# hongfz16/AvatarCLIP

Measured on NVIDIA H100. Metric: appearance-optim steps/sec (512 rays x 128 samples, CLIP loss), higher is better.
Workload: dtype bf16x3(split)->f32

## Files before the change

### avatarclip_b200/csrc/avc_gemm_tc.cuh

```cuda
#pragma once
#include <type_traits>
#include <cuda.h>
#include <cuda_bf16.h>

#include <cstdlib>

#include "avc_common.cuh"
#include "avc_wgmma.cuh"

namespace avc {
namespace tc {

__device__ __forceinline__ uint32_t smem_u32(const void* p) { return (uint32_t)__cvta_generic_to_shared(p); }

__device__ __forceinline__ void mbar_init(uint32_t bar, uint32_t count) {
  asm volatile("mbarrier.init.shared::cta.b64 [%0], %1;" ::"r"(bar), "r"(count));
}
__device__ __forceinline__ void mbar_expect_tx(uint32_t bar, uint32_t bytes) {
  asm volatile("mbarrier.arrive.expect_tx.shared::cta.b64 _, [%0], %1;" ::"r"(bar), "r"(bytes) : "memory");
}
__device__ __forceinline__ void mbar_arrive(uint32_t bar) {
  asm volatile("mbarrier.arrive.shared::cta.b64 _, [%0];" ::"r"(bar) : "memory");
}
__device__ __forceinline__ void mbar_wait(uint32_t bar, uint32_t parity) {
  uint32_t done = 0;
  for (uint32_t spins = 0; !done; ++spins) {
    asm volatile(
        "{\n\t.reg .pred p;\n\t"
        "mbarrier.try_wait.parity.shared::cta.b64 p, [%1], %2;\n\t"
        "selp.u32 %0, 1, 0, p;\n\t}"
        : "=r"(done) : "r"(bar), "r"(parity) : "memory");
    if (spins > (1u << 26)) __trap();
  }
}
constexpr int kNtProbeSlots = 9;
#ifdef AVC_NT_PROBE
static __device__ unsigned long long g_nt_probe[16][kNtProbeSlots];
#define AVC_PROBE(...) __VA_ARGS__
#define AVC_PROBE_WAIT(acc, bar, par) do { long long t__ = clock64(); mbar_wait(bar, par); (acc) += clock64() - t__; } while (0)
#define AVC_PROBE_ADD(id, slot, v) atomicAdd(&g_nt_probe[id][slot], (unsigned long long)(v))
#else
#define AVC_PROBE(...)
#define AVC_PROBE_WAIT(acc, bar, par) mbar_wait(bar, par)
#define AVC_PROBE_ADD(id, slot, v)
#endif
template <typename E, typename = void>
struct EpiProbeId { static constexpr int value = 0; };
template <typename E>
struct EpiProbeId<E, std::void_t<decltype(E::kProbeId)>> { static constexpr int value = E::kProbeId; };

__device__ __forceinline__ void pdl_wait() { asm volatile("griddepcontrol.wait;" ::: "memory"); }
__device__ __forceinline__ void pdl_trigger() { asm volatile("griddepcontrol.launch_dependents;" ::: "memory"); }
template <typename... KArgs, typename... Args>
static inline cudaError_t launch_pdl(void (*kern)(KArgs...), dim3 grid, dim3 block, size_t smem, cudaStream_t st, Args... args) {
  cudaLaunchConfig_t cfg{};
  cfg.gridDim = grid; cfg.blockDim = block; cfg.dynamicSmemBytes = smem; cfg.stream = st;
  cudaLaunchAttribute at[1];
  at[0].id = cudaLaunchAttributeProgrammaticStreamSerialization;
  at[0].val.programmaticStreamSerializationAllowed = 1;
  const char* e = getenv("AVC_TC_PDL");
  const int on = (e && atoi(e) == 0) ? 0 : 1;
  cfg.attrs = at; cfg.numAttrs = on ? 1 : 0;
  return cudaLaunchKernelEx(&cfg, kern, static_cast<KArgs>(args)...);
}

__device__ __forceinline__ void fence_barrier_init() { asm volatile("fence.mbarrier_init.release.cluster;" ::: "memory"); }
__device__ __forceinline__ void fence_proxy_async() { asm volatile("fence.proxy.async.shared::cta;" ::: "memory"); }
__device__ __forceinline__ void named_bar_sync(int id, int count) {
  asm volatile("bar.sync %0, %1;" ::"r"(id), "r"(count) : "memory");
}
__device__ __forceinline__ void named_bar_arrive(int id, int count) {
  asm volatile("bar.arrive %0, %1;" ::"r"(id), "r"(count) : "memory");
}

__device__ __forceinline__ void tma_load_2d(uint32_t dst, const CUtensorMap* map, int x, int y, uint32_t bar) {
  asm volatile(
      "cp.async.bulk.tensor.2d.shared::cluster.global.tile.mbarrier::complete_tx::bytes [%0], [%1, {%3, %4}], [%2];"
      ::"r"(dst), "l"((uint64_t)map), "r"(bar), "r"(x), "r"(y) : "memory");
}
__device__ __forceinline__ void tma_prefetch_desc(const CUtensorMap* map) {
  asm volatile("prefetch.tensormap [%0];" ::"l"((uint64_t)map) : "memory");
}

typedef CUresult (*PFN_encodeTiled)(CUtensorMap*, CUtensorMapDataType, cuuint32_t, void*, const cuuint64_t*,
                                    const cuuint64_t*, const cuuint32_t*, const cuuint32_t*, CUtensorMapInterleave,
                                    CUtensorMapSwizzle, CUtensorMapL2promotion, CUtensorMapFloatOOBfill);

static inline PFN_encodeTiled get_encode_fn() {
  static PFN_encodeTiled fn = nullptr;
  if (!fn) {
    void* p = nullptr;
    cudaDriverEntryPointQueryResult q;
    if (cudaGetDriverEntryPoint("cuTensorMapEncodeTiled", &p, cudaEnableDefault, &q) == cudaSuccess && p) fn = (PFN_encodeTiled)p;
  }
  return fn;
}

struct MapCacheEntry { const void* base; uint64_t rows, cols, ld; uint32_t bc, br; CUtensorMap map; };
static inline int make_map_bf16(CUtensorMap* m, const void* base, uint64_t rows, uint64_t cols, uint64_t ld,
                                uint32_t box_cols, uint32_t box_rows);
static inline int make_map_bf16_cached(CUtensorMap* m, const void* base, uint64_t rows, uint64_t cols, uint64_t ld,
                                       uint32_t box_cols, uint32_t box_rows) {
  static thread_local MapCacheEntry cache[256];
  uint64_t h = ((uintptr_t)base >> 8) * 0x9E3779B97F4A7C15ull ^ (rows * 31 + cols * 131 + ld * 7 + box_cols + 3 * box_rows);
  MapCacheEntry& e = cache[(h >> 32) & 255];
  if (e.base == base && e.rows == rows && e.cols == cols && e.ld == ld && e.bc == box_cols && e.br == box_rows) {
    *m = e.map;
    return 0;
  }
  int r = make_map_bf16(m, base, rows, cols, ld, box_cols, box_rows);
  if (r == 0) { e.base = base; e.rows = rows; e.cols = cols; e.ld = ld; e.bc = box_cols; e.br = box_rows; e.map = *m; }
  return r;
}
static inline int make_map_bf16(CUtensorMap* m, const void* base, uint64_t rows, uint64_t cols, uint64_t ld,
                                uint32_t box_cols, uint32_t box_rows) {
  PFN_encodeTiled fn = get_encode_fn();
  if (!fn) return AVC_E_BADCFG;
  if (((uintptr_t)base & 15u) || (ld * 2) % 16) return AVC_E_ALIGN;
  cuuint64_t dims[2] = {cols, rows};
  cuuint64_t strides[1] = {ld * 2};
  cuuint32_t box[2] = {box_cols, box_rows};
  cuuint32_t estr[2] = {1, 1};
  CUresult r = fn(m, CU_TENSOR_MAP_DATA_TYPE_BFLOAT16, 2, const_cast<void*>(base), dims, strides, box, estr,
                  CU_TENSOR_MAP_INTERLEAVE_NONE, CU_TENSOR_MAP_SWIZZLE_128B, CU_TENSOR_MAP_L2_PROMOTION_L2_256B,
                  CU_TENSOR_MAP_FLOAT_OOB_FILL_NONE);
  return r == CUDA_SUCCESS ? 0 : AVC_E_BADCFG;
}

static inline int make_map_rows_cached(CUtensorMap* m, int es, const void* base, uint64_t rows, uint64_t cols,
                                       uint64_t ld, uint32_t box_cols, uint32_t box_rows) {
  static thread_local MapCacheEntry cache[64];
  const uint64_t h = ((uintptr_t)base >> 8) * 0x9E3779B97F4A7C15ull ^ (rows * 31 + cols * 131 + ld * 7 + box_cols + 3 * box_rows + es);
  MapCacheEntry& e = cache[(h >> 32) & 63];
  const uint32_t bc = box_cols | ((uint32_t)es << 16);
  if (e.base == base && e.rows == rows && e.cols == cols && e.ld == ld && e.bc == bc && e.br == box_rows) {
    *m = e.map;
    return 0;
  }
  PFN_encodeTiled fn = get_encode_fn();
  if (!fn) return AVC_E_BADCFG;
  if (((uintptr_t)base & 15u) || (ld * es) % 16) return AVC_E_ALIGN;
  const uint32_t span = box_cols * es;
  const CUtensorMapSwizzle sw = span == 128 ? CU_TENSOR_MAP_SWIZZLE_128B : span == 64 ? CU_TENSOR_MAP_SWIZZLE_64B
                                                                                     : CU_TENSOR_MAP_SWIZZLE_32B;
  cuuint64_t dims[2] = {cols, rows};
  cuuint64_t strides[1] = {ld * es};
  cuuint32_t box[2] = {box_cols, box_rows};
  cuuint32_t estr[2] = {1, 1};
  CUresult r = fn(m, es == 4 ? CU_TENSOR_MAP_DATA_TYPE_FLOAT32 : CU_TENSOR_MAP_DATA_TYPE_BFLOAT16, 2, const_cast<void*>(base),
                  dims, strides, box, estr, CU_TENSOR_MAP_INTERLEAVE_NONE, sw, CU_TENSOR_MAP_L2_PROMOTION_L2_256B,
                  CU_TENSOR_MAP_FLOAT_OOB_FILL_NONE);
  if (r != CUDA_SUCCESS) return AVC_E_BADCFG;
  e.base = base; e.rows = rows; e.cols = cols; e.ld = ld; e.bc = bc; e.br = box_rows; e.map = *m;
  return 0;
}

struct SplitPtr {
  const __nv_bfloat16* hi;
  const __nv_bfloat16* lo;
  int ld;
};

constexpr int kBM = 128, kBK = 64;
constexpr int kConsumerThreads = 256;
constexpr int kTcThreads = kConsumerThreads + 32;
constexpr int kProducerWarp = kConsumerThreads / 32;
constexpr int kSmemMax = 232448;

constexpr int kNtBM = 64;
constexpr int kNtThreads = 384;
constexpr int kNtTurnBar = 1;

constexpr int kResK = 4;
constexpr int kEpiAStages = 3, kEpiSlotsMax = 8;
template <int BN, int NPROD, bool RESB = false, int EPI_SLOT = 0>
struct TcCfg {
  static constexpr int A_BYTES = kNtBM * kBK * 2;
  static constexpr int B_BYTES = BN * kBK * 2;
  static constexpr int NOP = (NPROD == 3) ? 2 : 1;
  static constexpr int BRES_BYTES = RESB ? kResK * NOP * B_BYTES : 0;
  static constexpr int STAGE_BYTES = RESB ? NOP * A_BYTES : NOP * (A_BYTES + B_BYTES);
  static constexpr int BAR_BYTES = EPI_SLOT ? 512 : 256;
  static constexpr int kBudget = kSmemMax - 1024  - BAR_BYTES - BRES_BYTES;
  static constexpr int STAGES = EPI_SLOT ? kEpiAStages : kBudget / STAGE_BYTES >= 8 ? 8 : kBudget / STAGE_BYTES;
  static constexpr int kEpiFit = EPI_SLOT ? (kBudget - STAGES * STAGE_BYTES) / (2 * EPI_SLOT) : 0;
  static constexpr int EPI_SLOTS = kEpiFit > kEpiSlotsMax ? kEpiSlotsMax : kEpiFit;
  static constexpr int SLOT_BYTES = EPI_SLOT;
  static constexpr int EPI_BYTES = 2 * EPI_SLOTS * EPI_SLOT;
  static constexpr int SMEM_BYTES = STAGES * STAGE_BYTES + BRES_BYTES + EPI_BYTES + 1024 + BAR_BYTES;
  static_assert(STAGES >= 2, "tile too large for shared memory");
  static_assert(!EPI_SLOT || EPI_SLOTS >= 2, "no room for two epilogue slots per consumer");
  static_assert(8 * (2 * STAGES + kResK + 4 * EPI_SLOTS) <= BAR_BYTES, "mbarriers overflow their area");
  static_assert(SMEM_BYTES <= kSmemMax, "exceeds the 227 KB of shared memory per CTA");
};

struct NoAux {};
template <typename E, typename = void>
struct EpiTraits {
  using Aux = NoAux;
  static __device__ __forceinline__ Aux prefetch(const E&, int, int) { return {}; }
  static __device__ __forceinline__ void apply(const E& e, int r, int c, float4 a, const Aux&) { e(r, c, a); }
};
template <typename E>
struct EpiTraits<E, std::void_t<typename E::Aux>> {
  using Aux = typename E::Aux;
  static __device__ __forceinline__ Aux prefetch(const E& e, int r, int c) { return e.prefetch(r, c); }
  static __device__ __forceinline__ void apply(const E& e, int r, int c, float4 a, const Aux& x) { e(r, c, a, x); }
};
template <typename E>
struct EpiBatch {
  static constexpr int kB = sizeof(typename EpiTraits<E>::Aux) > 16 ? 2 : 4;
  static constexpr int kCols = 8 * kB;
};

template <int E0, int E1 = 0, int E2 = 0>
struct Staged {
  static constexpr int kN = 1 + (E1 > 0) + (E2 > 0);
  static constexpr int kColBytes = E0 + E1 + E2;
  __host__ __device__ static constexpr int es(int i) { return i == 0 ? E0 : i == 1 ? E1 : E2; }
  __host__ __device__ static constexpr int before(int i) { return i == 0 ? 0 : i == 1 ? E0 : E0 + E1; }
};
struct StageOp { const void* base; int ld; int cols; };
template <typename E, typename = void>
struct EpiStage {
  static constexpr int kN = 0, kSlotBytes = 0;
};
template <typename E>
struct EpiStage<E, std::void_t<typename E::Stage>> {
  using S = typename E::Stage;
  static constexpr int kN = S::kN, kSlotBytes = kNtBM * EpiBatch<E>::kCols * S::kColBytes;
};
template <int N>
struct EpiMaps { CUtensorMap m[N]; };
template <>
struct EpiMaps<0> {};
template <int ES, int COLS>
__device__ __forceinline__ uint4 stage_read(uint32_t slab, int r, int c) {
  constexpr int kSpan = COLS * ES;
  static_assert(kSpan == 32 || kSpan == 64 || kSpan == 128, "swizzle span");
  const uint32_t lin = (uint32_t)(r * kSpan + c * ES);
  const uint32_t addr = slab + (lin ^ (((lin >> 7) & (kSpan / 16 - 1)) << 4));
  uint4 v = make_uint4(0u, 0u, 0u, 0u);
  if constexpr (ES == 4)
    asm volatile("ld.shared.v4.u32 {%0, %1, %2, %3}, [%4];" : "=r"(v.x), "=r"(v.y), "=r"(v.z), "=r"(v.w) : "r"(addr));
  else
    asm volatile("ld.shared.v2.u32 {%0, %1}, [%2];" : "=r"(v.x), "=r"(v.y) : "r"(addr));
  return v;
}
template <int ES>
__device__ __forceinline__ void l2_prefetch_tile(const void* base, int ld, int ncols, int m0, int n0, int bn, int M,
                                                 int et, int nth) {
  constexpr int kPerLine = 128 / ES;
  const int lpr = (bn + kPerLine - 1) / kPerLine;
  for (int i = et; i < kNtBM * lpr; i += nth) {
    const int row = m0 + i / lpr, col = n0 + (i % lpr) * kPerLine;
    if (row < M && col < ncols)
      asm volatile("prefetch.global.L2 [%0];" ::"l"(reinterpret_cast<const char*>(base) + ((size_t)row * ld + col) * ES));
  }
}
template <typename E, typename = void>
struct EpiL2 {
  static __device__ __forceinline__ void run(const E&, int, int, int, int, int, int) {}
};
template <typename E>
struct EpiL2<E, std::void_t<decltype(&E::l2_prefetch)>> {
  static __device__ __forceinline__ void run(const E& e, int m0, int n0, int bn, int M, int et, int nth) {
    if (m0 < M) e.l2_prefetch(m0, n0, bn, M, et, nth);
  }
};

struct EpiRing {
  uint32_t base;
  uint32_t full0, empty0;
  int q0;
  int r, c;
};
template <int BN, int SLOTS, typename Epi, typename MmaDone>
__device__ __forceinline__ void epilogue_nt(const Epi& epi, const float (&acc)[BN / 2], int row, int col0, int M, int N,
                                            int lane, MmaDone&& mma_done, const EpiRing& ring, long long& w_stage) {
  using Tr = EpiTraits<Epi>;
  const bool odd = lane & 1;
  constexpr int kB = EpiBatch<Epi>::kB, kNB = BN / 8 / kB;
  auto group = [&](int j) {
    const float s0 = odd ? acc[4 * j] : acc[4 * j + 2], s1 = odd ? acc[4 * j + 1] : acc[4 * j + 3];
    const float r0 = __shfl_xor_sync(0xffffffffu, s0, 1), r1 = __shfl_xor_sync(0xffffffffu, s1, 1);
    return odd ? make_float4(r0, r1, acc[4 * j + 2], acc[4 * j + 3]) : make_float4(acc[4 * j], acc[4 * j + 1], r0, r1);
  };
  if constexpr (EpiStage<Epi>::kN > 0) {
    using St = typename Epi::Stage;
    constexpr int kCols = EpiBatch<Epi>::kCols, kSlot = EpiStage<Epi>::kSlotBytes;
    mma_done();
#pragma unroll
    for (int b = 0; b < kNB; ++b) {
      const int q = ring.q0 + b, s = q % SLOTS;
      AVC_PROBE_WAIT(w_stage, ring.full0 + 8 * s, (q / SLOTS) & 1);
      const uint32_t slot = ring.base + s * kSlot;
      typename Tr::Aux aux[kB];
#pragma unroll
      for (int u = 0; u < kB; ++u) {
        uint4 raw[St::kN];
#pragma unroll
        for (int i = 0; i < St::kN; ++i) {
          const uint32_t slab = slot + kNtBM * kCols * St::before(i);
          raw[i] = St::es(i) == 4 ? stage_read<4, kCols>(slab, ring.r, ring.c + 8 * u)
                                  : stage_read<2, kCols>(slab, ring.r, ring.c + 8 * u);
        }
        aux[u] = Epi::from_stage(raw);
      }
#pragma unroll
      for (int u = 0; u < kB; ++u) {
        const int j = kB * b + u;
        const float4 v = group(j);
        const int col = col0 + 8 * j;
        if (row < M && col < N) Tr::apply(epi, row, col, v, aux[u]);
      }
      __syncwarp();
      if ((lane & 31) == 0) mbar_arrive(ring.empty0 + 8 * s);
    }
  } else {
    typename Tr::Aux aux[2][kB];
    auto load = [&](int b) {
#pragma unroll
      for (int u = 0; u < kB; ++u) {
        const int col = col0 + 8 * (kB * b + u);
        if (row < M && col < N) aux[b & 1][u] = Tr::prefetch(epi, row, col);
      }
    };
    load(0);
    mma_done();
#pragma unroll
    for (int b = 0; b < kNB; ++b) {
      if (b + 1 < kNB) load(b + 1);
#pragma unroll
      for (int u = 0; u < kB; ++u) {
        const int j = kB * b + u;
        const float s0 = odd ? acc[4 * j] : acc[4 * j + 2], s1 = odd ? acc[4 * j + 1] : acc[4 * j + 3];
        const float r0 = __shfl_xor_sync(0xffffffffu, s0, 1), r1 = __shfl_xor_sync(0xffffffffu, s1, 1);
        const float4 v = odd ? make_float4(r0, r1, acc[4 * j + 2], acc[4 * j + 3]) : make_float4(acc[4 * j], acc[4 * j + 1], r0, r1);
        const int col = col0 + 8 * j;
        if (row < M && col < N) Tr::apply(epi, row, col, v, aux[b & 1][u]);
      }
    }
  }
}

template <int BN, int NPROD, bool RESB, typename Epi>
__global__ void __launch_bounds__(kNtThreads, 1)
gemm_tc_nt_kernel(const __grid_constant__ CUtensorMap mapAhi, const __grid_constant__ CUtensorMap mapAlo,
                  const __grid_constant__ CUtensorMap mapBhi, const __grid_constant__ CUtensorMap mapBlo,
                  int M, int N, int K, Epi epi, int b_const, const __grid_constant__ EpiMaps<EpiStage<Epi>::kN> emaps) {
  using Cfg = TcCfg<BN, NPROD, RESB, EpiStage<Epi>::kSlotBytes>;
  constexpr int kStaged = EpiStage<Epi>::kN;
  constexpr int kEpiCols = EpiBatch<Epi>::kCols, kEpiNB = BN / kEpiCols;
  extern __shared__ uint8_t smem_raw[];
  uint8_t* smem = (uint8_t*)(((uintptr_t)smem_raw + 1023) & ~(uintptr_t)1023);
  constexpr int kOpBytes = Cfg::STAGES * Cfg::STAGE_BYTES + Cfg::BRES_BYTES + Cfg::EPI_BYTES;
  uint64_t* bars = (uint64_t*)(smem + kOpBytes);
  const uint32_t smem_base = smem_u32(smem);
  const uint32_t bres_base = smem_base + Cfg::STAGES * Cfg::STAGE_BYTES;
  const uint32_t full0 = smem_u32(bars), empty0 = full0 + 8 * Cfg::STAGES, bfull = empty0 + 8 * Cfg::STAGES;
  constexpr int kEpiOff = Cfg::STAGES * Cfg::STAGE_BYTES + Cfg::BRES_BYTES;
  const uint32_t efull0 = bfull + 8 * kResK, eempty0 = efull0 + 16 * Cfg::EPI_SLOTS;

  const int warp = threadIdx.x >> 5, lane = threadIdx.x & 31;
  const int tiles_n = (N + BN - 1) / BN;
  const int tiles_m = (M + kNtBM - 1) / kNtBM;
  const int nk = (K + kBK - 1) / kBK;
  const int n0 = (int)(blockIdx.x % tiles_n) * BN;
  const int m_first = (int)(blockIdx.x / tiles_n), m_stride = (int)(gridDim.x / tiles_n);
  const int n_tiles = m_first < tiles_m ? (tiles_m - m_first + m_stride - 1) / m_stride : 0;

  if (threadIdx.x == 0) {
    tma_prefetch_desc(&mapAhi); tma_prefetch_desc(&mapBhi);
    if (NPROD == 3) { tma_prefetch_desc(&mapAlo); tma_prefetch_desc(&mapBlo); }
    for (int s = 0; s < Cfg::STAGES; ++s) { mbar_init(full0 + 8 * s, 1); mbar_init(empty0 + 8 * s, 1); }
    for (int kb = 0; kb < kResK; ++kb) mbar_init(bfull + 8 * kb, 1);
    if constexpr (kStaged > 0) {
      for (int i = 0; i < kStaged; ++i) tma_prefetch_desc(&emaps.m[i]);
      for (int s = 0; s < 2 * Cfg::EPI_SLOTS; ++s) { mbar_init(efull0 + 8 * s, 1); mbar_init(eempty0 + 8 * s, 4); }
    }
    fence_barrier_init();
  }
  __syncthreads();

  if (warp < 4) {
    asm volatile("setmaxnreg.dec.sync.aligned.u32 40;");
    if constexpr (kStaged > 0) {
      if (threadIdx.x == 32 || threadIdx.x == 64) {
        const int c = warp - 1;
        pdl_wait();
        int q = 0;
        for (int j = c; j < n_tiles; j += 2) {
          const int m0 = (m_first + j * m_stride) * kNtBM;
#pragma unroll 1
          for (int b = 0; b < kEpiNB; ++b, ++q) {
            const int s = c * Cfg::EPI_SLOTS + q % Cfg::EPI_SLOTS;
            mbar_wait(eempty0 + 8 * s, ((q / Cfg::EPI_SLOTS) & 1) ^ 1);
            const uint32_t dst = smem_base + kEpiOff + s * Cfg::SLOT_BYTES;
            mbar_expect_tx(efull0 + 8 * s, (uint32_t)Cfg::SLOT_BYTES);
#pragma unroll
            for (int i = 0; i < kStaged; ++i)
              tma_load_2d(dst + kNtBM * kEpiCols * Epi::Stage::before(i), &emaps.m[i], n0 + b * kEpiCols, m0, efull0 + 8 * s);
          }
        }
        return;
      }
    }
    if (threadIdx.x == 0) {
      if (!b_const) pdl_wait();
      if (RESB && m_first < tiles_m) {
        for (int kb = 0; kb < nk; ++kb) {
          const uint32_t dst = bres_base + kb * (Cfg::NOP * Cfg::B_BYTES);
          mbar_expect_tx(bfull + 8 * kb, (uint32_t)(Cfg::NOP * Cfg::B_BYTES));
          tma_load_2d(dst, &mapBhi, kb * kBK, n0, bfull + 8 * kb);
          if (NPROD == 3) tma_load_2d(dst + Cfg::B_BYTES, &mapBlo, kb * kBK, n0, bfull + 8 * kb);
        }
      }
      if (b_const) pdl_wait();
      pdl_trigger();
      int it = 0;
      AVC_PROBE(long long w_empty = 0; const long long t_tma0 = clock64());
      for (int mt = m_first; mt < tiles_m; mt += m_stride) {
        const int m0 = mt * kNtBM;
        for (int kb = 0; kb < nk; ++kb, ++it) {
          const int s = it % Cfg::STAGES;
          AVC_PROBE_WAIT(w_empty, empty0 + 8 * s, ((it / Cfg::STAGES) & 1) ^ 1);
          const uint32_t st = smem_base + s * Cfg::STAGE_BYTES;
          mbar_expect_tx(full0 + 8 * s, Cfg::STAGE_BYTES);
          tma_load_2d(st, &mapAhi, kb * kBK, m0, full0 + 8 * s);
          if (NPROD == 3) tma_load_2d(st + Cfg::A_BYTES, &mapAlo, kb * kBK, m0, full0 + 8 * s);
          if (!RESB) {
            tma_load_2d(st + Cfg::NOP * Cfg::A_BYTES, &mapBhi, kb * kBK, n0, full0 + 8 * s);
            if (NPROD == 3) tma_load_2d(st + Cfg::NOP * Cfg::A_BYTES + Cfg::B_BYTES, &mapBlo, kb * kBK, n0, full0 + 8 * s);
          }
        }
      }
      AVC_PROBE_ADD(EpiProbeId<Epi>::value, 0, w_empty);
      AVC_PROBE_ADD(EpiProbeId<Epi>::value, 1, clock64() - t_tma0);
      AVC_PROBE_ADD(EpiProbeId<Epi>::value, 7, 1);
    }
    return;
  }

  asm volatile("setmaxnreg.inc.sync.aligned.u32 232;");
  const int c = (warp >> 2) - 1, wq = warp & 3;
  const int tw = threadIdx.x & 127;
  const bool leader = tw == 0;
  const int row_in = 16 * wq + (lane >> 2) + 8 * (lane & 1), col_in = 4 * ((lane >> 1) & 1);
  pdl_wait();
  float acc[BN / 2];
  long long w_stage = 0;
  EpiRing ring{smem_base + kEpiOff + c * Cfg::EPI_SLOTS * Cfg::SLOT_BYTES, efull0 + 8 * c * Cfg::EPI_SLOTS,
               eempty0 + 8 * c * Cfg::EPI_SLOTS, 0, row_in, col_in};
  AVC_PROBE(long long w_full = 0, w_turn = 0, t_mma = 0, t_epi = 0; const long long t_loop0 = clock64());
  EpiL2<Epi>::run(epi, (m_first + c * m_stride) * kNtBM, n0, BN, M, tw, 128);
  for (int j = c; j < n_tiles; j += 2) {
    const int m0 = (m_first + j * m_stride) * kNtBM;
    EpiL2<Epi>::run(epi, m0 + 2 * m_stride * kNtBM, n0, BN, M, tw, 128);
    AVC_PROBE(const long long t_turn0 = clock64());
    if (j > 0) named_bar_sync(kNtTurnBar + c, 256);
    AVC_PROBE(const long long t_mma0 = clock64(); w_turn += t_mma0 - t_turn0);
    int prev = -1, last = 0;
    for (int kb = 0; kb < nk; ++kb) {
      const int it = j * nk + kb, s = it % Cfg::STAGES;
      if (RESB && j < 2) mbar_wait(bfull + 8 * kb, 0);
      AVC_PROBE_WAIT(w_full, full0 + 8 * s, (it / Cfg::STAGES) & 1);
      const uint32_t a_hi = smem_base + s * Cfg::STAGE_BYTES;
      const uint32_t b_hi = RESB ? bres_base + kb * (Cfg::NOP * Cfg::B_BYTES) : smem_base + s * Cfg::STAGE_BYTES + Cfg::NOP * Cfg::A_BYTES;
      const uint64_t da = make_wgmma_desc(a_hi, 16, 1024), db = make_wgmma_desc(b_hi, 16, 1024);
      constexpr uint64_t kLoA = (uint64_t)(Cfg::A_BYTES >> 4), kLoB = (uint64_t)(Cfg::B_BYTES >> 4);
      wgmma_fence_acc(acc);
      wgmma_fence();
#pragma unroll
      for (int k4 = 0; k4 < kBK / 16; ++k4) {
        wgmma_bf16<BN, 0, 0>(acc, da + 2 * k4, db + 2 * k4, (kb | k4) ? 1u : 0u);
        if (NPROD == 3) {
          wgmma_bf16<BN, 0, 0>(acc, da + 2 * k4, db + kLoB + 2 * k4, 1u);
          wgmma_bf16<BN, 0, 0>(acc, da + kLoA + 2 * k4, db + 2 * k4, 1u);
        }
      }
      wgmma_commit();
      wgmma_fence_acc(acc);
      last = s;
      if (kb + 1 < nk) {
        wgmma_wait<1>();
        if (prev >= 0 && leader) mbar_arrive(empty0 + 8 * prev);
        prev = s;
      }
    }
    if (j + 1 < n_tiles) named_bar_arrive(kNtTurnBar + (c ^ 1), 256);
    ring.q0 = (j >> 1) * kEpiNB;
    epilogue_nt<BN, Cfg::EPI_SLOTS>(epi, acc, m0 + row_in, n0 + col_in, M, N, lane, [&] {
      wgmma_wait<0>();
      wgmma_fence_acc(acc);
      if (leader) {
        if (prev >= 0) mbar_arrive(empty0 + 8 * prev);
        mbar_arrive(empty0 + 8 * last);
      }
      AVC_PROBE(t_mma += clock64() - t_mma0);
    }, ring, w_stage);
    AVC_PROBE(t_epi += clock64() - t_mma0);
  }
  (void)w_stage;
  AVC_PROBE(if (leader) {
    AVC_PROBE_ADD(EpiProbeId<Epi>::value, 8, w_stage);
    AVC_PROBE_ADD(EpiProbeId<Epi>::value, 2, w_full);
    AVC_PROBE_ADD(EpiProbeId<Epi>::value, 3, w_turn);
    AVC_PROBE_ADD(EpiProbeId<Epi>::value, 4, t_mma);
    AVC_PROBE_ADD(EpiProbeId<Epi>::value, 5, t_epi - t_mma);
    AVC_PROBE_ADD(EpiProbeId<Epi>::value, 6, clock64() - t_loop0);
  })
}

template <int BN, int NPROD, bool RESB, typename Epi>
static inline int launch_gemm_tc_nt_bn(cudaStream_t st, int64_t M, int N, int K, const SplitPtr& A, const SplitPtr& B,
                                       const Epi& epi, bool b_const) {
  using Cfg = TcCfg<BN, NPROD, RESB, EpiStage<Epi>::kSlotBytes>;
  EpiMaps<EpiStage<Epi>::kN> emaps;
  if constexpr (EpiStage<Epi>::kN > 0) {
    for (int i = 0; i < EpiStage<Epi>::kN; ++i) {
      const StageOp op = epi.stage_op(i);
      if (!op.base) return AVC_E_BADCFG;
      AVC_TRY(make_map_rows_cached(&emaps.m[i], Epi::Stage::es(i), op.base, (uint64_t)M, (uint64_t)op.cols,
                                   (uint64_t)op.ld, EpiBatch<Epi>::kCols, kNtBM));
    }
  }
  CUtensorMap mAh, mAl, mBh, mBl;
  AVC_TRY(make_map_bf16_cached(&mAh, A.hi, (uint64_t)M, (uint64_t)K, (uint64_t)A.ld, kBK, kNtBM));
  AVC_TRY(make_map_bf16_cached(&mBh, B.hi, (uint64_t)N, (uint64_t)K, (uint64_t)B.ld, kBK, BN));
  if (NPROD == 3) {
    AVC_TRY(make_map_bf16_cached(&mAl, A.lo, (uint64_t)M, (uint64_t)K, (uint64_t)A.ld, kBK, kNtBM));
    AVC_TRY(make_map_bf16_cached(&mBl, B.lo, (uint64_t)N, (uint64_t)K, (uint64_t)B.ld, kBK, BN));
  } else {
    mAl = mAh; mBl = mBh;
  }
  auto kern = gemm_tc_nt_kernel<BN, NPROD, RESB, Epi>;
  static thread_local bool attr_set = false;
  if (!attr_set) {
    AVC_CUDA_TRY(cudaFuncSetAttribute(kern, cudaFuncAttributeMaxDynamicSharedMemorySize, Cfg::SMEM_BYTES));
    attr_set = true;
  }
  static thread_local int num_sms = 0;
  if (!num_sms) {
    int dev = 0;
    AVC_CUDA_TRY(cudaGetDevice(&dev));
    AVC_CUDA_TRY(cudaDeviceGetAttribute(&num_sms, cudaDevAttrMultiProcessorCount, dev));
  }
  const int tiles_n = ceil_div(N, BN);
  const int ntiles = ceil_div(M, kNtBM) * tiles_n;
  int g = ntiles < num_sms ? ntiles : num_sms;
  g = (g / tiles_n) * tiles_n;
  if (g < tiles_n) return AVC_E_BADCFG;
  dim3 grid(g);
  AVC_CUDA_TRY(launch_pdl(kern, dim3(grid), dim3(kNtThreads), (size_t)Cfg::SMEM_BYTES, st, mAh, mAl, mBh, mBl, (int)M, N, K, epi, b_const ? 1 : 0, emaps));
  AVC_LAUNCH_TRY();
  return 0;
}

template <int NPROD, typename Epi>
static inline int launch_gemm_tc_nt(cudaStream_t st, int64_t M, int N, int K, const SplitPtr& A, const SplitPtr& B,
                                    const Epi& epi, bool b_const = false) {
  if (M <= 0 || N <= 0) return 0;
  if (K <= kResK * kBK) {
    if (N <= 64) return launch_gemm_tc_nt_bn<64, NPROD, true, Epi>(st, M, N, K, A, B, epi, b_const);
    return launch_gemm_tc_nt_bn<128, NPROD, true, Epi>(st, M, N, K, A, B, epi, b_const);
  }
  if (N <= 64) return launch_gemm_tc_nt_bn<64, NPROD, false, Epi>(st, M, N, K, A, B, epi, b_const);
  return launch_gemm_tc_nt_bn<128, NPROD, false, Epi>(st, M, N, K, A, B, epi, b_const);
}

template <int BN, int NPROD>
struct TcTnCfg {
  static constexpr int BLK = kBK * 128;
  static constexpr int A_BYTES = (kBM / 64) * BLK;
  static constexpr int B_BYTES = (BN / 64) * BLK;
  static constexpr int NOP = (NPROD == 3) ? 2 : 1;
  static constexpr int STAGE_BYTES = NOP * (A_BYTES + B_BYTES);
  static constexpr int kBudget = kSmemMax - 1024  - 1024  - 256 ;
  static constexpr int STAGES = kBudget / STAGE_BYTES >= 4 ? 4 : kBudget / STAGE_BYTES;
  static constexpr int SMEM_BYTES = STAGES * STAGE_BYTES + 1024 + 1024 + 256;
  static_assert(SMEM_BYTES <= kSmemMax, "exceeds the 227 KB of shared memory per CTA");
  static_assert(STAGES >= 2, "tile too large for shared memory");
};

template <int BN, int NPROD>
__global__ void __launch_bounds__(kTcThreads, 1)
gemm_tc_tn_kernel(const __grid_constant__ CUtensorMap mapAhi, const __grid_constant__ CUtensorMap mapAlo,
                  const __grid_constant__ CUtensorMap mapBhi, const __grid_constant__ CUtensorMap mapBlo,
                  int P, int N1, int N2, int rows_per_split, float* __restrict__ C, int ldc,
                  float* __restrict__ colsum ) {
  using Cfg = TcTnCfg<BN, NPROD>;
  extern __shared__ uint8_t smem_raw[];
  uint8_t* smem = (uint8_t*)(((uintptr_t)smem_raw + 1023) & ~(uintptr_t)1023);
  uint8_t* ones_tile = smem + Cfg::STAGES * Cfg::STAGE_BYTES;
  uint64_t* bars = (uint64_t*)(ones_tile + 1024);
  const bool do_colsum = (colsum != nullptr) && (blockIdx.y == 0);
  const uint32_t smem_base = smem_u32(smem);
  const uint32_t full0 = smem_u32(bars), empty0 = full0 + 8 * Cfg::STAGES;

  const int warp = threadIdx.x >> 5, lane = threadIdx.x & 31;
  const int i0 = blockIdx.x * kBM, j0 = blockIdx.y * BN;
  const int p_begin = blockIdx.z * rows_per_split;
  const int p_end = min(P, p_begin + rows_per_split);
  const int nk = (p_end - p_begin + kBK - 1) / kBK;

  if (warp == kProducerWarp && lane == 0) {
    tma_prefetch_desc(&mapAhi); tma_prefetch_desc(&mapBhi);
    for (int s = 0; s < Cfg::STAGES; ++s) { mbar_init(full0 + 8 * s, 1); mbar_init(empty0 + 8 * s, 2); }
    fence_barrier_init();
  }
  if (do_colsum) {
    for (int i = threadIdx.x; i < 1024 / 4; i += blockDim.x) reinterpret_cast<uint32_t*>(ones_tile)[i] = 0x3F803F80u;
    fence_proxy_async();
  }
  __syncthreads();

  if (warp == kProducerWarp) {
    if (lane == 0) {
      pdl_wait();
      pdl_trigger();
      for (int kb = 0; kb < nk; ++kb) {
        const int s = kb % Cfg::STAGES;
        mbar_wait(empty0 + 8 * s, ((kb / Cfg::STAGES) & 1) ^ 1);
        const uint32_t st = smem_base + s * Cfg::STAGE_BYTES;
        const int p0 = p_begin + kb * kBK;
        mbar_expect_tx(full0 + 8 * s, Cfg::STAGE_BYTES);
#pragma unroll
        for (int a = 0; a < kBM / 64; ++a) {
          tma_load_2d(st + a * Cfg::BLK, &mapAhi, i0 + 64 * a, p0, full0 + 8 * s);
          if (NPROD == 3) tma_load_2d(st + Cfg::A_BYTES + a * Cfg::BLK, &mapAlo, i0 + 64 * a, p0, full0 + 8 * s);
        }
#pragma unroll
        for (int b = 0; b < BN / 64; ++b) {
          tma_load_2d(st + Cfg::NOP * Cfg::A_BYTES + b * Cfg::BLK, &mapBhi, j0 + 64 * b, p0, full0 + 8 * s);
          if (NPROD == 3)
            tma_load_2d(st + Cfg::NOP * Cfg::A_BYTES + Cfg::B_BYTES + b * Cfg::BLK, &mapBlo, j0 + 64 * b, p0, full0 + 8 * s);
        }
      }
    }
  } else {
    const int g = warp >> 2, wq = warp & 3;
    const bool leader = (threadIdx.x & 127) == 0;
    const uint64_t dones = make_wgmma_desc(smem_u32(ones_tile), 16, 1024);
    float acc[BN / 2], cs[4];
    int prev = -1;
    for (int kb = 0; kb < nk; ++kb) {
      const int s = kb % Cfg::STAGES;
      mbar_wait(full0 + 8 * s, (kb / Cfg::STAGES) & 1);
      const uint32_t a_hi = smem_base + s * Cfg::STAGE_BYTES + (uint32_t)g * Cfg::BLK;
      const uint32_t b_hi = smem_base + s * Cfg::STAGE_BYTES + Cfg::NOP * Cfg::A_BYTES;
      const uint64_t da = make_wgmma_desc(a_hi, Cfg::BLK, 1024), db = make_wgmma_desc(b_hi, Cfg::BLK, 1024);
      constexpr uint64_t kLoA = (uint64_t)(Cfg::A_BYTES >> 4), kLoB = (uint64_t)(Cfg::B_BYTES >> 4);
      wgmma_fence_acc(acc);
      wgmma_fence_acc(cs);
      auto batch = [&](auto with_colsum) {
        wgmma_fence();
#pragma unroll
        for (int k4 = 0; k4 < kBK / 16; ++k4) {
          wgmma_bf16<BN, 1, 1>(acc, da + 128 * k4, db + 128 * k4, (kb | k4) ? 1u : 0u);
          if (NPROD == 3) {
            wgmma_bf16<BN, 1, 1>(acc, da + 128 * k4, db + kLoB + 128 * k4, 1u);
            wgmma_bf16<BN, 1, 1>(acc, da + kLoA + 128 * k4, db + 128 * k4, 1u);
          }
          if constexpr (decltype(with_colsum)::value) {
            wgmma_bf16<8, 1, 0>(cs, da + 128 * k4, dones, (kb | k4) ? 1u : 0u);
            if (NPROD == 3) wgmma_bf16<8, 1, 0>(cs, da + kLoA + 128 * k4, dones, 1u);
          }
        }
        wgmma_commit();
      };
      if (do_colsum) batch(std::true_type{});
      else batch(std::false_type{});
      wgmma_fence_acc(acc);
      wgmma_fence_acc(cs);
      wgmma_wait<1>();
      if (prev >= 0 && leader) mbar_arrive(empty0 + 8 * prev);
      prev = s;
    }
    wgmma_wait<0>();
    wgmma_fence_acc(acc);
    wgmma_fence_acc(cs);
    if (leader) mbar_arrive(empty0 + 8 * prev);
    pdl_wait();
    const int r0 = i0 + 64 * g + 16 * wq + (lane >> 2);
#pragma unroll
    for (int j = 0; j < BN / 8; ++j) {
      const int c = j0 + 8 * j + 2 * (lane & 3);
#pragma unroll
      for (int h = 0; h < 2; ++h) {
        const int r = r0 + 8 * h;
        if (r < N1) {
          if (c < N2) atomicAdd(C + (size_t)r * ldc + c, acc[4 * j + 2 * h]);
          if (c + 1 < N2) atomicAdd(C + (size_t)r * ldc + c + 1, acc[4 * j + 2 * h + 1]);
        }
      }
    }
    if (do_colsum && (lane & 3) == 0) {
      if (r0 < N1) atomicAdd(colsum + r0, cs[0]);
      if (r0 + 8 < N1) atomicAdd(colsum + r0 + 8, cs[2]);
    }
  }
}

template <int NPROD>
static inline int launch_gemm_tc_tn(cudaStream_t st, int64_t P, int N1, int N2, const SplitPtr& A, const SplitPtr& B,
                                    float* C, int ldc, float* colsum = nullptr) {
  if (P <= 0 || N1 <= 0 || N2 <= 0) return 0;
  CUtensorMap mAh, mAl, mBh, mBl;
  AVC_TRY(make_map_bf16_cached(&mAh, A.hi, (uint64_t)P, (uint64_t)N1, (uint64_t)A.ld, 64, kBK));
  AVC_TRY(make_map_bf16_cached(&mBh, B.hi, (uint64_t)P, (uint64_t)N2, (uint64_t)B.ld, 64, kBK));
  if (NPROD == 3) {
    AVC_TRY(make_map_bf16_cached(&mAl, A.lo, (uint64_t)P, (uint64_t)N1, (uint64_t)A.ld, 64, kBK));
    AVC_TRY(make_map_bf16_cached(&mBl, B.lo, (uint64_t)P, (uint64_t)N2, (uint64_t)B.ld, 64, kBK));
  } else {
    mAl = mAh; mBl = mBh;
  }
  const int t1 = ceil_div(N1, kBM);
  auto go = [&](auto kern, int BN, int smem) -> int {
    AVC_CUDA_TRY(cudaFuncSetAttribute(kern, cudaFuncAttributeMaxDynamicSharedMemorySize, smem));
    const int t2 = ceil_div(N2, BN);
    static thread_local int sms = 0;
    if (!sms) { int dev = 0; AVC_CUDA_TRY(cudaGetDevice(&dev)); AVC_CUDA_TRY(cudaDeviceGetAttribute(&sms, cudaDevAttrMultiProcessorCount, dev)); }
    int splits = (sms + t1 * t2 - 1) / (t1 * t2);
    int rows = (int)round_up(ceil_div(P, splits), kBK);
    splits = ceil_div(P, rows);
    dim3 grid(t1, t2, splits);
    AVC_CUDA_TRY(launch_pdl(kern, grid, dim3(kTcThreads), (size_t)smem, st, mAh, mAl, mBh, mBl, (int)P, N1, N2, rows, C, ldc, colsum));
    AVC_LAUNCH_TRY();
    return 0;
  };
  if (N2 <= 64) return go(gemm_tc_tn_kernel<64, NPROD>, 64, TcTnCfg<64, NPROD>::SMEM_BYTES);
  if (N2 <= 128) return go(gemm_tc_tn_kernel<128, NPROD>, 128, TcTnCfg<128, NPROD>::SMEM_BYTES);
  return go(gemm_tc_tn_kernel<256, NPROD>, 256, TcTnCfg<256, NPROD>::SMEM_BYTES);
}

static __global__ void k_split_bf16(const float* __restrict__ src, int64_t rows, int cols, int ld_src,
                             __nv_bfloat16* __restrict__ hi, __nv_bfloat16* __restrict__ lo, int ld_dst) {
  int64_t i = (int64_t)blockIdx.x * blockDim.x + threadIdx.x;
  if (i >= rows * ld_dst) return;
  int64_t r = i / ld_dst;
  int c = (int)(i - r * ld_dst);
  float v = c < cols ? src[(size_t)r * ld_src + c] : 0.f;
  __nv_bfloat16 h = __float2bfloat16_rn(v);
  hi[i] = h;
  lo[i] = __float2bfloat16_rn(v - __bfloat162float(h));
}

}
}
```

### avatarclip_b200/csrc/avc_neus.cu

```cuda
#include <cstdio>
#include <cstring>

#include "avc_chain.h"
#include "avc_common.cuh"
#include "avc_gemm_simt.cuh"
#include "avc_gemm_tc.cuh"
#include "avc_neus_kernels.cuh"
#include "avc_neus_plan.cuh"

using namespace avc;

namespace {

inline int blocks_for(int64_t n, int threads) { return (int)((n + threads - 1) / threads); }

inline Split16 with_ld(Split16 s, int ld) { s.ld = ld; return s; }

template <int NP = 3, typename Epi>
int gemm_nt(const NeusPlan& pl, const NeusWs& w, cudaStream_t st, int64_t M, int N, int K, const float* A, int lda,
            const Split16& A16, int64_t pk_off, int ldb, const Epi& epi) {
  if (pl.cfg.engine == 1) {
    tc::SplitPtr a{A16.hi, A16.lo, lda}, b{w.pk_hi + pk_off, w.pk_lo + pk_off, ldb};
    return tc::launch_gemm_tc_nt<NP, Epi>(st, M, N, K, a, b, epi,  true);
  }
// ... 270 lines not shown
  return 0;
}

struct ChunkIO {
  const float *rays_o, *rays_d, *background;
  int bg_kind;
  float cos_anneal;
  int64_t Rc;
  avc_neus_outputs out;
};

CompositeArgs make_composite_args(const NeusPlan& pl, const NeusWs& w, const ChunkIO& io) {
  CompositeArgs A;
  A.rays_d = io.rays_d; A.z_vals = io.out.z_vals; A.sdf = w.sdf; A.cin = w.cin; A.rgb6 = w.rgb6;
  A.background = io.background; A.bg_kind = io.bg_kind; A.ctx = w.ctx; A.cos_anneal = io.cos_anneal;
  A.sample_dist = 2.0f / (float)pl.n0;
  A.S = pl.S; A.Rc = io.Rc;
  return A;
}

int composite_forward(const CompositeArgs& A, const avc_neus_outputs& out, float* ray_part, float* ctx,
                      cudaStream_t st) {
  k_composite_fwd<<<blocks_for(A.Rc, 8), 256, 0, st>>>(A, out.color_fine, out.extra_color_fine, out.s_val, out.cdf_fine,
                                                       out.weight_sum, out.weight_max, out.weights, ray_part);
  AVC_LAUNCH_TRY();
  k_reduce_ray_part<<<1, 1024, 0, st>>>(ray_part, A.Rc, 0, ctx + CTX_EIK_NUM);
  k_reduce_ray_part<<<1, 1024, 0, st>>>(ray_part, A.Rc, 1, ctx + CTX_EIK_DEN);
  AVC_LAUNCH_TRY();
  return 0;
}

int composite_backward(const CompositeArgs& A, const CompositeBwdArgs& G, float* ctx, cudaStream_t st) {
  k_composite_bwd<<<blocks_for(A.Rc, 8), 256, 0, st>>>(A, G);
  AVC_LAUNCH_TRY();
  k_reduce_ray_part<<<1, 1024, 0, st>>>(G.ray_part, A.Rc, 2, ctx + CTX_INVS_BAR);
  AVC_LAUNCH_TRY();
  return 0;
}

int relax_count(const float* rays_o, const float* rays_d, const float* z_vals, int S, int64_t Rc, float sample_dist,
                float* ray_part, float* ctx, cudaStream_t st) {
  k_relax_count<<<blocks_for(Rc, 8), 256, 0, st>>>(rays_o, rays_d, z_vals, S, Rc, sample_dist, ray_part);
  k_reduce_ray_part<<<1, 1024, 0, st>>>(ray_part, Rc, 1, ctx + CTX_EIK_DEN);
  AVC_LAUNCH_TRY();
  return 0;
}

int ctx_init(const float* params, int64_t off_var, float* ctx, int zero_sums, cudaStream_t st) {
  k_ctx_init<<<1, 32, 0, st>>>(params, off_var, ctx, zero_sums);
  AVC_LAUNCH_TRY();
  return 0;
}

int finalize_fwd(const float* ctx, float* gerr_out, cudaStream_t st) {
  k_finalize_fwd<<<1, 32, 0, st>>>(ctx, gerr_out);
  AVC_LAUNCH_TRY();
  return 0;
}

int variance_grad(const float* params, int64_t off_var, const float* ctx, const float* g_sval, int64_t R,
                  float* grad_var, cudaStream_t st) {
  k_variance_grad<<<1, 256, 0, st>>>(params, off_var, ctx, g_sval, R, grad_var);
  AVC_LAUNCH_TRY();
  return 0;
}

int fine_forward(const NeusPlan& pl, const NeusWs& w, const ChunkIO& io, bool write_outputs, cudaStream_t st) {
  const int64_t P = io.Rc * pl.S;
  const float* pack = w.pack;
  EncodeTargets t = make_targets(pl, w);
  k_encode_fine<<<blocks_for(P * 8, 256), 256, 0, st>>>(io.rays_o, io.rays_d, io.out.z_vals, pl.S, io.Rc,
                                                    2.0f / (float)pl.n0, pl.cfg.sdf_scale, pl.cfg.sdf_multires, pl.E,
                                                    pl.EP, w.cin, write_outputs ? io.out.mid_z_vals : nullptr,
                                                    write_outputs ? io.out.inside_sphere : nullptr, t);
  AVC_LAUNCH_TRY();
  AVC_TRY(value_chain(pl, w, P, true, true, w.sdf, st));
  AVC_TRY(gradient_chain(pl, w, P, write_outputs ? io.out.gradients : nullptr, st));
  {
    const LinDim& c0 = pl.col[0];
    const bool tc1 = pl.cfg.engine == 1;
    const Split16 none16{nullptr, nullptr, 0};
    EpiColor0 e0{pack + c0.pk_b, w.cin, pack + pl.pk_c0xT, pl.Hc, (tc1 && 1 < pl.Lc) ? nullptr : w.ch[1], pl.Hc,
                 (tc1 && 1 == pl.Lc) ? none16 : w.ch16[1]};
    AVC_TRY(gemm_nt_color(pl, w, st, P, pl.Hc, pl.F, w.feat, pl.Fp, w.feat16, c0.pk_W, pl.Fp, e0));
    for (int l = 1; l < pl.Lc; ++l) {
      const LinDim& c = pl.col[l];
      EpiRelu e{pack + c.pk_b, (tc1 && l + 1 < pl.Lc) ? nullptr : w.ch[l + 1], pl.Hc,
                (tc1 && l + 1 == pl.Lc) ? none16 : w.ch16[l + 1]};
      AVC_TRY(gemm_nt_color(pl, w, st, P, pl.Hc, pl.Hc, w.ch[l], pl.Hc, w.ch16[l], c.pk_W, pl.Hc, e));
    }
    OutHeads oh{w.rgb6};
    k_thin_nt<6, OutHeads><<<blocks_for(P, 8 * kThinPPW), 256, 0, st>>>(w.ch[pl.Lc], pl.Hc, pl.Hc, pack + pl.pk_W6, pl.Hc,
                                                             pack + pl.pk_b6, P, oh);
    AVC_LAUNCH_TRY();
  }
  if (write_outputs) AVC_TRY(composite_forward(make_composite_args(pl, w, io), io.out, w.ray_part, w.ctx, st));
  return 0;
}

template <int NI>
int thin_tn(cudaStream_t st, const float* S, int lds, float s_scale, const float* Hm, int ldh, int NC, int64_t P,
            float* out, int si, int sc, float* bout, int split = NI, float* out2 = nullptr, float* bout2 = nullptr) {
  const int rows = 128;
  k_thin_tn<NI><<<blocks_for(P, rows), 256, 0, st>>>(S, lds, s_scale, Hm, ldh, NC, P, rows, out, si, sc, bout, split,
                                                     out2, bout2);
  AVC_LAUNCH_TRY();
  return 0;
}

int colsum(cudaStream_t st, const float* X, int ld, int NC, int64_t P, float scale, float* out) {
  const int rows = 64;
  k_colsum<<<blocks_for(P, rows), 256, 0, st>>>(X, ld, NC, P, rows, scale, out);
  AVC_LAUNCH_TRY();
  return 0;
}

int fine_backward(const NeusPlan& pl, const NeusWs& w, const ChunkIO& io, const avc_neus_cotangents& cot,
                  cudaStream_t st) {
  const int64_t P = io.Rc * pl.S;
  const float* pack = w.pack;
  float* wbar = w.wbar;
  CompositeArgs A = make_composite_args(pl, w, io);
  CompositeBwdArgs G;
  G.g_color = cot.color_fine; G.g_extra = cot.extra_color_fine; G.g_wsum = cot.weight_sum; G.g_wmax = cot.weight_max;
  G.g_w = cot.weights; G.g_cdf = cot.cdf_fine; G.g_n = cot.gradients; G.g_gerr = cot.gradient_error;
  G.weights = io.out.weights;
  G.y6bar = w.y6bar; G.sdfbar = w.sdfbar; G.nbar = w.nbar; G.ray_part = w.ray_part;
  AVC_TRY(composite_backward(A, G, w.ctx, st));

  {
    const LinDim& dh = pl.col[pl.Lc];
    const LinDim& dx = pl.extra;
    AVC_TRY(thin_tn<6>(st, w.y6bar, 8, 1.f, w.ch[pl.Lc], pl.Hc, pl.Hc, P, wbar + dh.off_v, pl.Hc, 1, wbar + dh.off_b, 3,
                       wbar + dx.off_v, wbar + dx.off_b));
    k_heads_dgrad<<<blocks_for(P * pl.Hc / 4, 256), 256, 0, st>>>(w.y6bar, pack + pl.pk_W6, pl.Hc, w.ch[pl.Lc], P,
                                                              (pl.cfg.engine == 1 && pl.Lc > 1) ? nullptr : w.cbar[0],
                                                              w.cbar16[0]);
    AVC_LAUNCH_TRY();
  }
  int cur = 0;
  for (int l = pl.Lc - 1; l >= 0; --l) {
    const LinDim& c = pl.col[l];
    float* cb = w.cbar[cur];
    if (l > 0) {
      AVC_TRY(gemm_tn(pl, w, st, P, pl.Hc, pl.Hc, cb, pl.Hc, w.cbar16[cur], w.ch[l], pl.Hc, w.ch16[l], wbar + c.off_v, c.K,
                      wbar + c.off_b, color_single(pl)));
      const bool tc1 = pl.cfg.engine == 1;
      EpiDgradRelu e{tc1 ? nullptr : w.ch[l], w.ch16[l].hi, (tc1 && l > 1) ? nullptr : w.cbar[cur ^ 1], pl.Hc,
                     w.cbar16[cur ^ 1]};
      AVC_TRY(gemm_nt_color(pl, w, st, P, pl.Hc, pl.Hc, cb, pl.Hc, w.cbar16[cur], c.pk_WT, pl.Hc, e));
      cur ^= 1;
    } else {
      AVC_TRY(gemm_tn(pl, w, st, P, pl.Hc, pl.F, cb, pl.Hc, w.cbar16[cur], w.feat, pl.Fp, w.feat16, wbar + c.off_v + 6, c.K,
                      wbar + c.off_b, color_single(pl)));
      AVC_TRY(thin_tn<6>(st, w.cin, 8, 1.f, cb, pl.Hc, pl.Hc, P, wbar + c.off_v, 1, c.K, nullptr));
      EpiStore es{pl.cfg.engine == 1 ? nullptr : w.featbar, pl.Fp, pl.F, w.featbar16};
      AVC_TRY(gemm_nt_color(pl, w, st, P, pl.F, pl.Hc, cb, pl.Hc, w.cbar16[cur], c.pk_WT, pl.Hc, es));
      OutNbarAdd on{w.nbar};
      k_thin_nt<6, OutNbarAdd><<<blocks_for(P, 8 * kThinPPW), 256, 0, st>>>(cb, pl.Hc, pl.Hc, pack + pl.pk_c0xT, pl.Hc, nullptr,
                                                                 P, on);
      AVC_LAUNCH_TRY();
    }
  }

  int ucur = 0;
  {
    const LinDim& d0 = pl.sdf[0];
    k_dge<<<blocks_for(P * 8, 256), 256, 0, st>>>(w.cin, w.nbar, pl.EP, pl.E, pl.cfg.sdf_multires, pl.cfg.sdf_scale, P,
                                                  pl.cfg.engine == 1 ? nullptr : w.ubar[0], d0.Kp, w.gebar,
                                                  with_ld(w.ubar16[0], d0.Kp));
    AVC_LAUNCH_TRY();
  }
  for (int l = 0; l <= pl.L; ++l) {
    const LinDim& d = pl.sdf[l];
    float* ub = w.ubar[ucur];
    if (l == pl.L) {
      AVC_TRY(colsum(st, ub, d.Kp, d.K, P, 1.f, wbar + d.off_v));
      break;
    }
    const Split16 ub16 = with_ld(w.ubar16[ucur], d.Kp);
    AVC_TRY(gemm_tn(pl, w, st, P, d.N, d.K, w.qt[l], d.Np, w.qt16[l], ub, d.Kp, ub16, wbar + d.off_v, d.K));
    const LinDim& dn = pl.sdf[l + 1];
    EpiChainBwd e;
    e.N = d.N; e.Np = d.Np; e.D1 = w.z[l]; e.QT = pl.cfg.engine == 1 ? nullptr : w.qt[l]; e.qt16 = w.qt16[l];
    e.ZBAR = w.zbar[l];
    e.UNEXT = (pl.cfg.engine == 1 && l + 1 < pl.L) ? nullptr : w.ubar[ucur ^ 1];
    e.ldu = dn.Kp; e.s_next = dn.skip ? kSqrtHalf : 1.f;
    const Split16 unext16 = (pl.cfg.engine == 1 && l + 1 == pl.L) ? Split16{nullptr, nullptr, 0} : with_ld(w.ubar16[ucur ^ 1], dn.Kp);
    e.u16 = unext16;
    AVC_TRY(gemm_nt(pl, w, st, P, d.N, d.K, ub, d.Kp, ub16, d.pk_W, d.Kp, e));
    if (dn.skip) {
      k_fill_gebar<<<blocks_for(P * pl.E, 256), 256, 0, st>>>(w.gebar, pl.EP, pl.E, P, w.ubar[ucur ^ 1], dn.Kp,
                                                              dn.K - pl.E, unext16);
      AVC_LAUNCH_TRY();
    }
    ucur ^= 1;
  }

  {
    const LinDim& dL = pl.sdf[pl.L];
    const float inv_scale = 1.0f / pl.cfg.sdf_scale;
    AVC_TRY(thin_tn<1>(st, w.sdfbar, 1, inv_scale, w.in[pl.L], dL.Kp, dL.K, P, wbar + dL.off_v, 0, 1, wbar + dL.off_b));
    AVC_TRY(gemm_tn(pl, w, st, P, pl.F, dL.K, w.featbar, pl.Fp, w.featbar16, w.in[pl.L], dL.Kp, w.in16[pl.L],
                    wbar + dL.off_v + dL.K, dL.K, wbar + dL.off_b + 1));
    const LinDim& dp = pl.sdf[pl.L - 1];
    EpiDgrad e;
    e.Nprev = dp.N; e.Npp = dp.Np; e.s = dL.skip ? kSqrtHalf : 1.f;
    e.D1prev = w.z[pl.L - 1]; e.ZBARprev = w.zbar[pl.L - 1];
    e.sdfbar = w.sdfbar; e.wsdf = pack + pl.pk_wsdf; e.sdf_inv_scale = inv_scale;
    e.z16 = w.zbar16[pl.L - 1]; e.store_f32 = pl.cfg.engine != 1;
    AVC_TRY(gemm_nt(pl, w, st, P, dp.N, pl.F, w.featbar, pl.Fp, w.featbar16, dL.pk_WT, pl.Fp, e));
  }
  for (int l = pl.L - 1; l >= 0; --l) {
    const LinDim& d = pl.sdf[l];
    AVC_TRY(gemm_tn(pl, w, st, P, d.N, d.K, w.zbar[l], d.Np, w.zbar16[l], w.in[l], d.Kp, w.in16[l], wbar + d.off_v, d.K,
                    wbar + d.off_b));
    if (l == 0) break;
    const LinDim& dp = pl.sdf[l - 1];
    EpiDgrad e;
    e.Nprev = dp.N; e.Npp = dp.Np; e.s = d.skip ? kSqrtHalf : 1.f;
    e.D1prev = w.z[l - 1]; e.ZBARprev = w.zbar[l - 1];
    e.sdfbar = nullptr; e.wsdf = nullptr; e.sdf_inv_scale = 1.f;
    e.z16 = w.zbar16[l - 1]; e.store_f32 = pl.cfg.engine != 1;
    AVC_TRY(gemm_nt(pl, w, st, P, dp.N, d.N, w.zbar[l], d.Np, w.zbar16[l], d.pk_WT, d.Np, e));
  }
  return 0;
}

int weight_norm_backward_all(const NeusPlan& pl, const float* params, const float* wbar, float* grads,
                             cudaStream_t st) {
  WnJobs jobs;
  jobs.n = 0;
  int maxN = 1;
  auto one = [&](const LinDim& d) {
    jobs.j[jobs.n++] = WnJob{params + d.off_v, params + d.off_g, wbar + d.off_v, wbar + d.off_b, d.N, d.K,
                             grads + d.off_g, grads + d.off_v, grads + d.off_b};
    if (d.N > maxN) maxN = d.N;
  };
  for (int l = 0; l <= pl.L; ++l) one(pl.sdf[l]);
  for (int l = 0; l <= pl.Lc; ++l) one(pl.col[l]);
  one(pl.extra);
  k_wn_backward<<<dim3(maxN, jobs.n), 128, 0, st>>>(jobs);
  AVC_LAUNCH_TRY();
  return 0;
}

int check_ptr16(const void* p) { return ((uintptr_t)p & 15u) ? AVC_E_ALIGN : 0; }

avc_neus_outputs offset_outputs(const avc_neus_outputs& o, int64_t r0, int S) {
  avc_neus_outputs q = o;
  q.color_fine += r0 * 3; q.extra_color_fine += r0 * 3; q.s_val += r0; q.cdf_fine += r0 * S;
  q.weight_sum += r0; q.weight_max += r0; q.gradients += r0 * S * 3; q.weights += r0 * S;
  q.mid_z_vals += r0 * S; q.inside_sphere += r0 * S; q.z_vals += r0 * S;
  return q;
}

avc_neus_cotangents offset_cot(const avc_neus_cotangents& c, int64_t r0, int S) {
  avc_neus_cotangents q = c;
  if (q.color_fine) q.color_fine += r0 * 3;
  if (q.extra_color_fine) q.extra_color_fine += r0 * 3;
  if (q.s_val) q.s_val += r0;
  if (q.cdf_fine) q.cdf_fine += r0 * S;
  if (q.weight_sum) q.weight_sum += r0;
  if (q.weight_max) q.weight_max += r0;
  if (q.gradients) q.gradients += r0 * S * 3;
  if (q.weights) q.weights += r0 * S;
  return q;
}

}

extern "C" {

int avc_abi_version(void) { return AVC_ABI_VERSION; }

int avc_nt_probe_read(unsigned long long* host_out, int reset) {
#ifdef AVC_NT_PROBE
  if (!host_out) return AVC_E_NULL;
  AVC_CUDA_TRY(cudaDeviceSynchronize());
  AVC_CUDA_TRY(cudaMemcpyFromSymbol(host_out, tc::g_nt_probe, sizeof(unsigned long long) * 16 * tc::kNtProbeSlots));
  if (reset) {
    static unsigned long long zeros[16 * tc::kNtProbeSlots];
    AVC_CUDA_TRY(cudaMemcpyToSymbol(tc::g_nt_probe, zeros, sizeof(zeros)));
  }
  return 0;
#else
  (void)host_out; (void)reset;
  return AVC_E_BADCFG;
#endif
}
const char* avc_build_arch(void) { return "sm_90a"; }

int avc_tc_epi_test(int32_t kind, const float* A, const float* B, int64_t M, int32_t N, int32_t K, int32_t Nv,
                    const float* X, float* Y, int32_t ldx, const float* v1, const float* v2, float s, float s2, float* OUT,
                    float* OUT2, int32_t ld2, void* workspace, size_t workspace_bytes, avc_stream_t stream) {
  if (!A || !B || !X || !workspace) return AVC_E_NULL;
  if (M <= 0 || N <= 0 || K <= 0 || ldx % 8 || ld2 % 8) return AVC_E_SIZE;
  const int ld = (int)round_up(K, 8);
  Carver cv(workspace);
  __nv_bfloat16* ah = cv.take<__nv_bfloat16>(M * ld);
  __nv_bfloat16* al = cv.take<__nv_bfloat16>(M * ld);
  __nv_bfloat16* bh = cv.take<__nv_bfloat16>((int64_t)N * ld);
  __nv_bfloat16* bl = cv.take<__nv_bfloat16>((int64_t)N * ld);
  __nv_bfloat16* xh = cv.take<__nv_bfloat16>(M * ldx);
  __nv_bfloat16* xl = cv.take<__nv_bfloat16>(M * ldx);
  if (cv.used() > workspace_bytes) return AVC_E_SIZE;
  cudaStream_t st = (cudaStream_t)stream;
  tc::k_split_bf16<<<blocks_for(M * ld, 256), 256, 0, st>>>(A, M, K, K, ah, al, ld);
  tc::k_split_bf16<<<blocks_for((int64_t)N * ld, 256), 256, 0, st>>>(B, N, K, K, bh, bl, ld);
  const float* xs = kind == 0 ? Y : X;
  if (kind == 0 || kind == 4) tc::k_split_bf16<<<blocks_for(M * ldx, 256), 256, 0, st>>>(xs, M, ldx, ldx, xh, xl, ldx);
  AVC_LAUNCH_TRY();
  const tc::SplitPtr a{ah, al, ld}, b{bh, bl, ld};
  const Split16 none{nullptr, nullptr, ldx};
  switch (kind) {
    case 0: {
      EpiChainBwd e;
      e.N = N; e.Np = ldx; e.D1 = X; e.QT = nullptr; e.qt16 = Split16{xh, xl, ldx}; e.ZBAR = OUT; e.UNEXT = OUT2;
      e.ldu = ld2; e.s_next = s; e.u16 = Split16{nullptr, nullptr, ld2};
      return tc::launch_gemm_tc_nt<3>(st, M, N, K, a, b, e);
    }
    case 1:
    case 2: {
      EpiDgrad e;
      e.Nprev = N; e.Npp = ldx; e.s = s; e.D1prev = X; e.ZBARprev = Y;
      e.sdfbar = kind == 2 ? v1 : nullptr; e.wsdf = kind == 2 ? v2 : nullptr; e.sdf_inv_scale = s2;
      e.z16 = none; e.store_f32 = 1;
      return tc::launch_gemm_tc_nt<3>(st, M, N, K, a, b, e);
    }
    case 3: {
      EpiChain e;
      e.Nprev = Nv; e.Npp = ldx; e.s = s; e.D1prev = X; e.QTprev = OUT; e.GE = OUT2; e.EP = ld2; e.E = N - Nv;
      e.q16 = none;
      return tc::launch_gemm_tc_nt<3>(st, M, N, K, a, b, e);
    }
    case 4: {
      EpiDgradRelu e{nullptr, xh, OUT, ldx, none};
      return tc::launch_gemm_tc_nt<3>(st, M, N, K, a, b, e);
    }
    case 5: {
      EpiGe e{OUT2, ld2, N};
      return tc::launch_gemm_tc_nt<3>(st, M, N, K, a, b, e);
    }
  }
  return AVC_E_BADCFG;
}

int avc_neus_kernel_test(int32_t kind, const int64_t* d, const float* fs, const void* const* in, void* const* out,
                         avc_stream_t stream) {
  if (!d || !fs || !in || !out) return AVC_E_NULL;
  cudaStream_t st = (cudaStream_t)stream;
  const auto F32 = [](const void* p) { return (const float*)p; };
  const auto O32 = [](void* p) { return (float*)p; };
  switch (kind) {
    case 0: return ctx_init(F32(in[0]), d[0], O32(out[0]), (int)d[1], st);
    case 1:
    case 2: {
      const int S = (int)d[0], bg_kind = (int)d[2];
      const int64_t Rc = d[1];
      if (S < 1 || S > 256 || Rc < 1) return AVC_E_SIZE;
      if (bg_kind < 0 || bg_kind > 2 || (bg_kind != 0 && !in[5])) return AVC_E_BADCFG;
      CompositeArgs A;
      A.rays_d = F32(in[0]); A.z_vals = F32(in[1]); A.sdf = F32(in[2]); A.cin = F32(in[3]); A.rgb6 = F32(in[4]);
      A.background = F32(in[5]); A.bg_kind = bg_kind; A.cos_anneal = fs[0]; A.sample_dist = fs[1]; A.S = S; A.Rc = Rc;
      if (kind == 1) {
        float* ctx = O32(out[8]);
        A.ctx = ctx;
        avc_neus_outputs o;
        memset(&o, 0, sizeof(o));
        o.color_fine = O32(out[0]); o.extra_color_fine = O32(out[1]); o.s_val = O32(out[2]); o.cdf_fine = O32(out[3]);
        o.weight_sum = O32(out[4]); o.weight_max = O32(out[5]); o.weights = O32(out[6]);
        return composite_forward(A, o, O32(out[7]), ctx, st);
      }
      float* ctx = O32(out[4]);
      A.ctx = ctx;
      CompositeBwdArgs G;
      G.g_color = F32(in[6]); G.g_extra = F32(in[7]); G.g_wsum = F32(in[8]); G.g_wmax = F32(in[9]);
      G.g_w = F32(in[10]); G.g_cdf = F32(in[11]); G.g_n = F32(in[12]); G.g_gerr = F32(in[13]); G.weights = F32(in[14]);
      if (G.g_wmax && !G.weights) return AVC_E_NULL;
      G.y6bar = O32(out[0]); G.sdfbar = O32(out[1]); G.nbar = O32(out[2]); G.ray_part = O32(out[3]);
      return composite_backward(A, G, ctx, st);
    }
    case 3: {
      if (d[0] < 1 || d[1] < 1) return AVC_E_SIZE;
      return relax_count(F32(in[0]), F32(in[1]), F32(in[2]), (int)d[0], d[1], fs[0], O32(out[0]), O32(out[1]), st);
    }
    case 4: return finalize_fwd(F32(in[0]), O32(out[0]), st);
    case 5: return variance_grad(F32(in[0]), d[0], F32(in[1]), F32(in[2]), d[1], O32(out[0]), st);
    case 6: {
      const int n = (int)d[0], pitch = (int)d[1], Rc = (int)d[2];
      if (n < 1 || pitch < n || Rc < 1) return AVC_E_SIZE;
      return coarse_z(F32(in[0]), F32(in[1]), F32(in[2]), n, pitch, Rc, O32(out[0]), st);
    }
    case 7: {
      const int n = (int)d[0], pitch = (int)d[1], Rc = (int)d[2], per = (int)d[3];
      if (n < 2 || n > kPlaceMaxN || pitch < n || Rc < 1 || per < 1 || per > kPlaceMaxNew) return AVC_E_SIZE;
      return upsample(F32(in[0]), F32(in[1]), F32(in[2]), F32(in[3]), n, pitch, Rc, fs[0], per, O32(out[0]), st);
    }
    case 8: {
      const int n = (int)d[0], pitch = (int)d[1], Rc = (int)d[2], per = (int)d[3], pitch_o = (int)d[4];
      if (n < 1 || n > kPlaceMaxN || pitch < n || Rc < 1 || per < 1 || per > kPlaceMaxNew || pitch_o < n + per)
        return AVC_E_SIZE;
      if (in[3] && !out[1]) return AVC_E_NULL;
      return merge(F32(in[0]), F32(in[1]), n, pitch, F32(in[2]), F32(in[3]), per, Rc, O32(out[0]), O32(out[1]), pitch_o,
                   st);
    }
  }
  return AVC_E_BADCFG;
}

int avc_neus_param_count(const avc_neus_cfg* cfg, int64_t* n_params) {
  if (!cfg || !n_params) return AVC_E_NULL;
  NeusPlan pl;
  AVC_TRY(build_plan(cfg, &pl));
  *n_params = pl.n_params;
  return 0;
}

int avc_neus_param_offset(const avc_neus_cfg* cfg, int net, int layer, int which, int64_t* offset, int64_t* numel) {
  if (!cfg || !offset || !numel) return AVC_E_NULL;
  NeusPlan pl;
  AVC_TRY(build_plan(cfg, &pl));
  const LinDim* d = nullptr;
  if (net == 0) { if (layer < 0 || layer > pl.L) return AVC_E_SIZE; d = &pl.sdf[layer]; }
  else if (net == 1) { if (layer < 0 || layer > pl.Lc) return AVC_E_SIZE; d = &pl.col[layer]; }
  else if (net == 2) d = &pl.extra;
  else if (net == 3) { *offset = pl.off_var; *numel = 1; return 0; }
  else return AVC_E_BADCFG;
  if (which == 0) { *offset = d->off_g; *numel = d->N; }
  else if (which == 1) { *offset = d->off_v; *numel = (int64_t)d->N * d->K; }
  else if (which == 2) { *offset = d->off_b; *numel = d->N; }
  else return AVC_E_BADCFG;
  return 0;
}

int avc_neus_workspace_bytes(const avc_neus_cfg* cfg, int64_t max_rays_per_chunk, size_t* bytes) {
  if (!cfg || !bytes) return AVC_E_NULL;
  if (max_rays_per_chunk <= 0) return AVC_E_SIZE;
  NeusPlan pl;
  AVC_TRY(build_plan(cfg, &pl));
  NeusWs w;
  carve_ws(pl, max_rays_per_chunk, nullptr, &w);
  *bytes = w.bytes;
  return 0;
}

int avc_neus_render_fwd(const avc_neus_cfg* cfg, const float* params, const float* rays_o, const float* rays_d,
                        const float* near, const float* far, const float* jitter, const float* background,
                        int bg_kind, const float* z_vals_in, float cos_anneal_ratio, int64_t R,
                        const avc_neus_outputs* out, void* workspace, size_t workspace_bytes,
                        int64_t max_rays_per_chunk, avc_stream_t stream) {
  if (!cfg || !params || !rays_o || !rays_d || !out || !workspace) return AVC_E_NULL;
  if (!z_vals_in && (!near || !far)) return AVC_E_NULL;
  if (!out->color_fine || !out->extra_color_fine || !out->s_val || !out->cdf_fine || !out->weight_sum ||
      !out->weight_max || !out->gradients || !out->weights || !out->mid_z_vals || !out->gradient_error ||
      !out->inside_sphere || !out->z_vals)
    return AVC_E_NULL;
  if (bg_kind < 0 || bg_kind > 2 || (bg_kind != 0 && !background)) return AVC_E_BADCFG;
  if (R <= 0 || max_rays_per_chunk <= 0) return AVC_E_SIZE;
  NeusPlan pl;
  AVC_TRY(build_plan(cfg, &pl));
  AVC_TRY(check_ptr16(workspace)); AVC_TRY(check_ptr16(params)); AVC_TRY(check_ptr16(out->z_vals));
  const int64_t Rc_max = R < max_rays_per_chunk ? R : max_rays_per_chunk;
  NeusWs w;
  carve_ws(pl, Rc_max, workspace, &w);
  if (w.bytes > workspace_bytes) return AVC_E_SIZE;
  cudaStream_t st = (cudaStream_t)stream;

  AVC_TRY(prepare_weights(pl, w, params, st));
  AVC_TRY(ctx_init(params, pl.off_var, w.ctx, 1, st));

  for (int64_t r0 = 0; r0 < R; r0 += Rc_max) {
    const int64_t Rc = (R - r0) < Rc_max ? (R - r0) : Rc_max;
    ChunkIO io;
    io.rays_o = rays_o + r0 * 3; io.rays_d = rays_d + r0 * 3;
    io.background = (bg_kind == 2) ? background + r0 : background;
    io.bg_kind = bg_kind; io.cos_anneal = cos_anneal_ratio; io.Rc = Rc;
    io.out = offset_outputs(*out, r0, pl.S);
    if (z_vals_in && z_vals_in + r0 * pl.S == io.out.z_vals) {
    } else if (z_vals_in) {
      AVC_CUDA_TRY(cudaMemcpyAsync(io.out.z_vals, z_vals_in + r0 * pl.S, sizeof(float) * Rc * pl.S,
                                   cudaMemcpyDeviceToDevice, st));
    } else {
      AVC_TRY(place_samples(pl, w, io.rays_o, io.rays_d, near + r0, far + r0, jitter ? jitter + r0 : nullptr,
                            (int)Rc, io.out.z_vals, st));
    }
    AVC_TRY(fine_forward(pl, w, io, true, st));
  }
  return finalize_fwd(w.ctx, out->gradient_error, st);
}

int avc_neus_render_bwd(const avc_neus_cfg* cfg, const float* params, const float* rays_o, const float* rays_d,
                        const float* background, int bg_kind, float cos_anneal_ratio, int64_t R,
                        const avc_neus_outputs* fwd_out, const avc_neus_cotangents* cot, float* grad_params,
                        void* workspace, size_t workspace_bytes, int64_t max_rays_per_chunk, int32_t flags,
                        avc_stream_t stream) {
  if (!cfg || !params || !rays_o || !rays_d || !fwd_out || !cot || !grad_params || !workspace) return AVC_E_NULL;
  if (!fwd_out->z_vals || !fwd_out->weights) return AVC_E_NULL;
  if (bg_kind < 0 || bg_kind > 2 || (bg_kind != 0 && !background)) return AVC_E_BADCFG;
  if (R <= 0 || max_rays_per_chunk <= 0) return AVC_E_SIZE;
  NeusPlan pl;
  AVC_TRY(build_plan(cfg, &pl));
  AVC_TRY(check_ptr16(workspace)); AVC_TRY(check_ptr16(params)); AVC_TRY(check_ptr16(grad_params));
  const int64_t Rc_max = R < max_rays_per_chunk ? R : max_rays_per_chunk;
  NeusWs w;
  carve_ws(pl, Rc_max, workspace, &w);
  if (w.bytes > workspace_bytes) return AVC_E_SIZE;
  cudaStream_t st = (cudaStream_t)stream;
  const bool single = (R <= Rc_max) && !(flags & AVC_BWD_RECOMPUTE);

  AVC_CUDA_TRY(cudaMemsetAsync(w.wbar, 0, sizeof(float) * (size_t)pl.n_params, st));
  AVC_TRY(ctx_init(params, pl.off_var, w.ctx, 1, st));
  for (int64_t r0 = 0; r0 < R; r0 += Rc_max) {
    const int64_t Rc = (R - r0) < Rc_max ? (R - r0) : Rc_max;
    AVC_TRY(relax_count(rays_o + r0 * 3, rays_d + r0 * 3, fwd_out->z_vals + r0 * pl.S, pl.S, Rc, 2.0f / (float)pl.n0,
                        w.ray_part, w.ctx, st));
  }
  if (!single) AVC_TRY(prepare_weights(pl, w, params, st));
  for (int64_t r0 = 0; r0 < R; r0 += Rc_max) {
    const int64_t Rc = (R - r0) < Rc_max ? (R - r0) : Rc_max;
    ChunkIO io;
    io.rays_o = rays_o + r0 * 3; io.rays_d = rays_d + r0 * 3;
    io.background = (bg_kind == 2) ? background + r0 : background;
    io.bg_kind = bg_kind; io.cos_anneal = cos_anneal_ratio; io.Rc = Rc;
    io.out = offset_outputs(*fwd_out, r0, pl.S);
    if (!single) AVC_TRY(fine_forward(pl, w, io, false, st));
    avc_neus_cotangents c = offset_cot(*cot, r0, pl.S);
    AVC_TRY(fine_backward(pl, w, io, c, st));
  }
  AVC_TRY(weight_norm_backward_all(pl, params, w.wbar, grad_params, st));
  return variance_grad(params, pl.off_var, w.ctx, cot->s_val, R, grad_params + pl.off_var, st);
}

int avc_neus_sdf_query(const avc_neus_cfg* cfg, const float* params, const float* pts, int64_t P, float* sdf_out,
                       void* workspace, size_t workspace_bytes, avc_stream_t stream) {
  if (!cfg || !params || !pts || !sdf_out || !workspace) return AVC_E_NULL;
  if (P <= 0) return AVC_E_SIZE;
  NeusPlan pl;
  AVC_TRY(build_plan(cfg, &pl));
  size_t one = 0;
  AVC_TRY(avc_neus_workspace_bytes(cfg, 1, &one));
  NeusWs w;
  int64_t Rc = 1;
  {
    NeusWs w2; carve_ws(pl, 2, nullptr, &w2);
    size_t per = w2.bytes - one;
    if (workspace_bytes < one) return AVC_E_SIZE;
    Rc = 1 + (int64_t)((workspace_bytes - one) / (per ? per : 1));
    while (Rc > 1) { carve_ws(pl, Rc, nullptr, &w); if (w.bytes <= workspace_bytes) break; --Rc; }
  }
  carve_ws(pl, Rc, workspace, &w);
  if (w.bytes > workspace_bytes) return AVC_E_SIZE;
  cudaStream_t st = (cudaStream_t)stream;
  AVC_TRY(prepare_weights(pl, w, params, st));
  const int64_t cap = Rc * pl.S;
  EncodeTargets t = make_targets(pl, w);
  for (int64_t p0 = 0; p0 < P; p0 += cap) {
    int64_t n = (P - p0) < cap ? (P - p0) : cap;
    k_encode_points<<<blocks_for(n * 8, 256), 256, 0, st>>>(pts + p0 * 3, n, pl.cfg.sdf_scale, pl.cfg.sdf_multires, pl.E,
                                                        pl.EP, t);
    AVC_LAUNCH_TRY();
    AVC_TRY(value_chain(pl, w, n, false, false, sdf_out + p0, st));
  }
  return 0;
}

namespace {
__global__ void k_points_to_cin(const float* __restrict__ pts, int64_t P, float* __restrict__ cin) {
  int64_t p = (int64_t)blockIdx.x * blockDim.x + threadIdx.x;
  if (p >= P) return;
  float4* c = reinterpret_cast<float4*>(cin + (size_t)p * 8);
  c[0] = make_float4(pts[p * 3], pts[p * 3 + 1], pts[p * 3 + 2], 0.f);
  c[1] = make_float4(0.f, 0.f, 0.f, 0.f);
}
__global__ void k_assemble_sdf_feat(const float* __restrict__ sdf, const float* __restrict__ feat, int Fp, int F, int64_t P,
                                    float* __restrict__ out) {
  int64_t i = (int64_t)blockIdx.x * blockDim.x + threadIdx.x;
  if (i >= P * (F + 1)) return;
  int64_t p = i / (F + 1);
  int c = (int)(i - p * (F + 1));
  out[i] = c == 0 ? sdf[p] : feat[(size_t)p * Fp + (c - 1)];
}
}

int avc_neus_sdf_eval(const avc_neus_cfg* cfg_in, const float* params, const float* pts, int64_t P, float* sdf_feat_out,
                      float* grad_out, void* workspace, size_t workspace_bytes, avc_stream_t stream) {
  if (!cfg_in || !params || !pts || !workspace) return AVC_E_NULL;
  if (!sdf_feat_out && !grad_out) return AVC_E_NULL;
  if (P <= 0) return AVC_E_SIZE;
  avc_neus_cfg cfg = *cfg_in;
  cfg.engine = 0;
  NeusPlan pl;
  AVC_TRY(build_plan(&cfg, &pl));
  size_t one = 0;
  AVC_TRY(avc_neus_workspace_bytes(&cfg, 1, &one));
  NeusWs w;
  int64_t Rc = 1;
  {
    NeusWs w2; carve_ws(pl, 2, nullptr, &w2);
    size_t per = w2.bytes - one;
    if (workspace_bytes < one) return AVC_E_SIZE;
    Rc = 1 + (int64_t)((workspace_bytes - one) / (per ? per : 1));
    while (Rc > 1) { carve_ws(pl, Rc, nullptr, &w); if (w.bytes <= workspace_bytes) break; --Rc; }
  }
  carve_ws(pl, Rc, workspace, &w);
  if (w.bytes > workspace_bytes) return AVC_E_SIZE;
  cudaStream_t st = (cudaStream_t)stream;
  AVC_TRY(prepare_weights(pl, w, params, st));
  const int64_t cap = Rc * pl.S;
  EncodeTargets t = make_targets(pl, w);
  for (int64_t p0 = 0; p0 < P; p0 += cap) {
    int64_t n = (P - p0) < cap ? (P - p0) : cap;
    k_encode_points<<<blocks_for(n * 8, 256), 256, 0, st>>>(pts + p0 * 3, n, pl.cfg.sdf_scale, pl.cfg.sdf_multires, pl.E,
                                                        pl.EP, t);
    k_points_to_cin<<<blocks_for(n, 256), 256, 0, st>>>(pts + p0 * 3, n, w.cin);
    AVC_LAUNCH_TRY();
    AVC_TRY(value_chain(pl, w, n, grad_out != nullptr, sdf_feat_out != nullptr, w.sdf, st));
    if (sdf_feat_out) {
      k_assemble_sdf_feat<<<blocks_for(n * (pl.F + 1), 256), 256, 0, st>>>(w.sdf, w.feat, pl.Fp, pl.F, n,
                                                                          sdf_feat_out + p0 * (pl.F + 1));
      AVC_LAUNCH_TRY();
    }
    if (grad_out) AVC_TRY(gradient_chain(pl, w, n, grad_out + p0 * 3, st));
  }
  return 0;
}

static double round_beta(float b) { return (double)((long long)((double)b * 1e6 + 0.5)) / 1e6; }

int avc_adam_step(float* params, const float* grads, float* exp_avg, float* exp_avg_sq, int64_t n, float lr,
                  float beta1, float beta2, float eps, int64_t step, float grad_scale, avc_stream_t stream) {
  if (!params || !grads || !exp_avg || !exp_avg_sq) return AVC_E_NULL;
  if (n <= 0 || step < 1) return AVC_E_SIZE;
  const double b1 = round_beta(beta1), b2 = round_beta(beta2);
  double bc1 = 1.0 - pow(b1, (double)step);
  double bc2 = 1.0 - pow(b2, (double)step);
  k_adam<<<blocks_for(n, 256), 256, 0, (cudaStream_t)stream>>>(params, grads, exp_avg, exp_avg_sq, n, lr, (float)b1,
                                                               (float)b2, eps, (float)bc1, (float)sqrt(bc2), grad_scale,
                                                               (float)(1.0 - b1), (float)(1.0 - b2));
  AVC_LAUNCH_TRY();
  return 0;
}

int avc_adam_step_dev(float* params, const float* grads, float* exp_avg, float* exp_avg_sq, int64_t n, float* state,
                      float beta1, float beta2, float eps, float grad_scale, avc_stream_t stream) {
// ... 13 lines not shown
```

### avatarclip_b200/csrc/avc_neus_kernels.cuh

```cuda
#pragma once
#include <cuda_bf16.h>

#include "avc_common.cuh"

namespace avc {

struct Split16 {
  __nv_bfloat16* hi; __nv_bfloat16* lo; int ld;
};
__device__ __forceinline__ void split16_put(const Split16& s, size_t row, int col, float v) {
  if (!s.hi) return;
  __nv_bfloat16 h = __float2bfloat16_rn(v);
  s.hi[row * s.ld + col] = h;
  s.lo[row * s.ld + col] = __float2bfloat16_rn(v - __bfloat162float(h));
}
__device__ __forceinline__ void split16_get4(uint2 hi, uint2 lo, float v[4]) {
  v[0] = __uint_as_float(hi.x << 16) + __uint_as_float(lo.x << 16);
  v[1] = __uint_as_float(hi.x & 0xffff0000u) + __uint_as_float(lo.x & 0xffff0000u);
  v[2] = __uint_as_float(hi.y << 16) + __uint_as_float(lo.y << 16);
  v[3] = __uint_as_float(hi.y & 0xffff0000u) + __uint_as_float(lo.y & 0xffff0000u);
}
__device__ __forceinline__ float split16_get(const Split16& s, size_t row, int col) {
  return __bfloat162float(s.hi[row * s.ld + col]) + __bfloat162float(s.lo[row * s.ld + col]);
}
// ... 278 lines not shown
      float t = __shfl_up_sync(0xffffffffu, inc, of);
      if (lane >= of) inc += t;
    }
    if (j < nsec) scdf[j + 1] = carry + inc;
    carry += __shfl_sync(0xffffffffu, inc, 31);
  }
  __syncwarp();
  const float ustart = 0.5f / (float)per, uend = 1.0f - 0.5f / (float)per;
  for (int t = lane; t < per; t += 32) {
    const float u = torch_linspace(ustart, uend, per, t);
    int lo = 0, hi = n;
    while (lo < hi) { int mid = (lo + hi) >> 1; if (scdf[mid] <= u) lo = mid + 1; else hi = mid; }
    const int below = max(lo - 1, 0), above = min(lo, n - 1);
    const float cb = scdf[below], ca = scdf[above], zb = sz[below], za = sz[above];
    float denom = __fsub_rn(ca, cb);
    if (denom < 1e-5f) denom = 1.0f;
    const float tt = __fdiv_rn(__fsub_rn(u, cb), denom);
    newz[(size_t)r * per + t] = __fadd_rn(zb, __fmul_rn(tt, __fsub_rn(za, zb)));
  }
}

__global__ void __launch_bounds__(256)
k_merge(const float* __restrict__ z, const float* __restrict__ sdf, int n, int pitch, const float* __restrict__ newz,
        const float* __restrict__ news, int per, int Rc, float* __restrict__ zo, float* __restrict__ so, int pitch_o) {
  __shared__ float s_z[8][kPlaceMaxN];
  __shared__ float s_n[8][kPlaceMaxNew];
  const int wib = threadIdx.x >> 5, lane = threadIdx.x & 31;
  const int r = blockIdx.x * 8 + wib;
  if (r >= Rc) return;
  float* sz = s_z[wib];
  float* sn = s_n[wib];
  for (int j = lane; j < n; j += 32) sz[j] = z[(size_t)r * pitch + j];
  for (int t = lane; t < per; t += 32) sn[t] = newz[(size_t)r * per + t];
  __syncwarp();
  for (int i = lane; i < n; i += 32) {
    const float v = sz[i];
    int lo = 0, hi = per;
    while (lo < hi) { int mid = (lo + hi) >> 1; if (sn[mid] < v) lo = mid + 1; else hi = mid; }
    zo[(size_t)r * pitch_o + i + lo] = v;
    if (news) so[(size_t)r * pitch_o + i + lo] = sdf[(size_t)r * pitch + i];
  }
  for (int t = lane; t < per; t += 32) {
    const float v = sn[t];
    int lo = 0, hi = n;
    while (lo < hi) { int mid = (lo + hi) >> 1; if (sz[mid] <= v) lo = mid + 1; else hi = mid; }
    zo[(size_t)r * pitch_o + t + lo] = v;
    if (news) so[(size_t)r * pitch_o + t + lo] = news[(size_t)r * per + t];
  }
}

constexpr int kThinPPW = 4;
template <int NI, typename Out>
__global__ void __launch_bounds__(256)
k_thin_nt(const float* __restrict__ A, int lda, int K, const float* __restrict__ W, int ldw,
          const float* __restrict__ b, int64_t P, Out out) {
  const int64_t p0 = ((int64_t)blockIdx.x * (blockDim.x >> 5) + (threadIdx.x >> 5)) * kThinPPW;
  if (p0 >= P) return;
  const int lane = threadIdx.x & 31;
  float acc[kThinPPW][NI];
#pragma unroll
  for (int j = 0; j < kThinPPW; ++j)
#pragma unroll
    for (int i = 0; i < NI; ++i) acc[j][i] = 0.f;
  for (int k = lane * 4; k < K; k += 128) {
    float4 a[kThinPPW];
#pragma unroll
    for (int j = 0; j < kThinPPW; ++j)
      a[j] = *reinterpret_cast<const float4*>(A + (size_t)(p0 + j < P ? p0 + j : p0) * lda + k);
#pragma unroll
    for (int i = 0; i < NI; ++i) {
      const float4 w = *reinterpret_cast<const float4*>(W + (size_t)i * ldw + k);
#pragma unroll
      for (int j = 0; j < kThinPPW; ++j)
        acc[j][i] = fmaf(a[j].x, w.x, fmaf(a[j].y, w.y, fmaf(a[j].z, w.z, fmaf(a[j].w, w.w, acc[j][i]))));
    }
  }
#pragma unroll
  for (int j = 0; j < kThinPPW; ++j)
#pragma unroll
    for (int i = 0; i < NI; ++i) acc[j][i] = warp_sum(acc[j][i]) + (b ? b[i] : 0.f);
#pragma unroll
  for (int j = 0; j < kThinPPW; ++j)
    if (lane == j && p0 + j < P) out(p0 + j, acc[j]);
}

struct OutSdf {
  float* sdf; float inv_scale; int nz; int pitch;
  __device__ void operator()(int64_t p, const float* v) const {
    int64_t o = nz > 0 ? (p / nz) * pitch + (p % nz) : p;
    sdf[o] = v[0] * inv_scale;
  }
};
struct OutHeads {
  float* rgb6;
  __device__ void operator()(int64_t p, const float* v) const {
    float4 a = make_float4(sigmoidf_acc(v[0]), sigmoidf_acc(v[1]), sigmoidf_acc(v[2]), sigmoidf_acc(v[3]));
    float4 b = make_float4(sigmoidf_acc(v[4]), sigmoidf_acc(v[5]), 0.f, 0.f);
    reinterpret_cast<float4*>(rgb6 + (size_t)p * 8)[0] = a;
    reinterpret_cast<float4*>(rgb6 + (size_t)p * 8)[1] = b;
  }
};
struct OutNbarAdd {
  float* nbar;
  __device__ void operator()(int64_t p, const float* v) const {
    nbar[(size_t)p * 4 + 0] += v[3]; nbar[(size_t)p * 4 + 1] += v[4]; nbar[(size_t)p * 4 + 2] += v[5];
  }
};

template <int NI>
__global__ void __launch_bounds__(256)
k_thin_tn(const float* __restrict__ S, int lds, float s_scale, const float* __restrict__ Hm, int ldh, int NC,
          int64_t P, int rows_per_block, float* __restrict__ out, int si, int sc, float* __restrict__ bout,
          int split, float* __restrict__ out2, float* __restrict__ bout2) {
  __shared__ float sS[64][NI];
  const int64_t p0 = (int64_t)blockIdx.x * rows_per_block;
  const int64_t p1 = min(P, p0 + (int64_t)rows_per_block);
  float bacc = 0.f;
  for (int cb = 0; cb < NC; cb += blockDim.x) {
    const int c = cb + threadIdx.x;
    float acc[NI];
#pragma unroll
    for (int i = 0; i < NI; ++i) acc[i] = 0.f;
    for (int64_t pb = p0; pb < p1; pb += 64) {
      int nr = (int)min((int64_t)64, p1 - pb);
      __syncthreads();
      for (int t = threadIdx.x; t < nr * NI; t += blockDim.x) {
        int rr = t / NI, ii = t % NI;
        sS[rr][ii] = S[(size_t)(pb + rr) * lds + ii] * s_scale;
      }
      __syncthreads();
      if (c < NC) {
        const float* hp = Hm + (size_t)pb * ldh + c;
        int rr = 0;
        for (; rr + 8 <= nr; rr += 8) {
          float h[8];
#pragma unroll
          for (int u = 0; u < 8; ++u) h[u] = hp[(size_t)(rr + u) * ldh];
#pragma unroll
          for (int u = 0; u < 8; ++u)
#pragma unroll
            for (int i = 0; i < NI; ++i) acc[i] = fmaf(sS[rr + u][i], h[u], acc[i]);
        }
        for (; rr < nr; ++rr) {
          float h = hp[(size_t)rr * ldh];
#pragma unroll
          for (int i = 0; i < NI; ++i) acc[i] = fmaf(sS[rr][i], h, acc[i]);
        }
      }
      if ((bout || bout2) && cb == 0 && threadIdx.x < NI)
        for (int rr = 0; rr < nr; ++rr) bacc += sS[rr][threadIdx.x];
    }
    if (c < NC) {
#pragma unroll
      for (int i = 0; i < NI; ++i) {
        float* o = (i < split) ? out + (size_t)i * si : out2 + (size_t)(i - split) * si;
        atomicAdd(o + (size_t)c * sc, acc[i]);
      }
    }
  }
  if (threadIdx.x < NI) {
    const int i = threadIdx.x;
    if (i < split) { if (bout) atomicAdd(bout + i, bacc); }
    else if (bout2) atomicAdd(bout2 + (i - split), bacc);
  }
}

__global__ void __launch_bounds__(256)
k_colsum(const float* __restrict__ X, int ld, int NC, int64_t P, int rows_per_block, float scale,
         float* __restrict__ out) {
  const int64_t p0 = (int64_t)blockIdx.x * rows_per_block;
  const int64_t p1 = min(P, p0 + (int64_t)rows_per_block);
  for (int c = threadIdx.x; c < NC; c += blockDim.x) {
    float a[8] = {0.f, 0.f, 0.f, 0.f, 0.f, 0.f, 0.f, 0.f};
    int64_t p = p0;
    for (; p + 7 < p1; p += 8) {
      float x[8];
#pragma unroll
      for (int u = 0; u < 8; ++u) x[u] = X[(size_t)(p + u) * ld + c];
#pragma unroll
      for (int u = 0; u < 8; ++u) a[u] += x[u];
    }
    for (; p < p1; ++p) a[0] += X[(size_t)p * ld + c];
    atomicAdd(out + c, (((a[0] + a[1]) + (a[2] + a[3])) + ((a[4] + a[5]) + (a[6] + a[7]))) * scale);
  }
}

__global__ void k_chain_start(const float* __restrict__ wsdf, int KL, int skipL, int E, int EP,
                              const float* __restrict__ zprev, int Nprev, int Npp, int64_t P,
                              float* __restrict__ qt, float* __restrict__ ge, Split16 qt16) {
  int64_t i4 = ((int64_t)blockIdx.x * blockDim.x + threadIdx.x) * 4;
  int64_t tot = P * (int64_t)Npp;
  if (i4 < tot) {
    int64_t p = i4 / Npp;
    int c = (int)(i4 - p * Npp);
    const float4 z = *reinterpret_cast<const float4*>(zprev + i4);
    const float zz[4] = {z.x, z.y, z.z, z.w};
    float v[4];
#pragma unroll
    for (int i = 0; i < 4; ++i)
      v[i] = (c + i < Nprev) ? zz[i] * wsdf[c + i] * (skipL ? kSqrtHalf : 1.f) : 0.f;
    if (qt) *reinterpret_cast<float4*>(qt + i4) = make_float4(v[0], v[1], v[2], v[3]);
    split16_put4(qt16, (size_t)p, c, v);
  }
  int64_t i = (int64_t)blockIdx.x * blockDim.x + threadIdx.x;
  if (i < P * (int64_t)EP) {
    int64_t p = i / EP;
    int e = (int)(i - p * EP);
    ge[i] = (skipL && e < E) ? wsdf[KL - E + e] * kSqrtHalf : 0.f;
  }
}

__global__ void k_normal(const float* __restrict__ ge, int EP, int multires, float scale, int64_t P,
                         float* __restrict__ cin, float* __restrict__ grad_out) {
  int64_t p = (int64_t)blockIdx.x * blockDim.x + threadIdx.x;
  if (p >= P) return;
  const float* g = ge + (size_t)p * EP;
  float* c = cin + (size_t)p * 8;
  float n[3];
#pragma unroll
  for (int a = 0; a < 3; ++a) {
    float y = c[a] * scale;
    float acc = g[a];
    float f = 1.f;
    for (int k = 0; k < multires; ++k) {
      float sn, cs;
      sincosf(y * f, &sn, &cs);
      acc += f * (cs * g[3 + 6 * k + a] - sn * g[6 + 6 * k + a]);
      f *= 2.f;
    }
    n[a] = acc;
  }
  c[3] = n[0]; c[4] = n[1]; c[5] = n[2];
  if (grad_out) { grad_out[p * 3 + 0] = n[0]; grad_out[p * 3 + 1] = n[1]; grad_out[p * 3 + 2] = n[2]; }
}

__global__ void k_dge(const float* __restrict__ cin, const float* __restrict__ nbar, int EP, int E, int multires,
                      float scale, int64_t P, float* __restrict__ ubar0, int ldu, float* __restrict__ gebar,
                      Split16 u16) {
  const int64_t t = (int64_t)blockIdx.x * blockDim.x + threadIdx.x;
  const int64_t p = t >> 3;
  const int gl = (int)(t & 7);
  if (p >= P) return;
  const float* c = cin + (size_t)p * 8;
  const float nb[3] = {nbar[p * 4 + 0], nbar[p * 4 + 1], nbar[p * 4 + 2]};
  float* u = ubar0 ? ubar0 + (size_t)p * ldu : nullptr;
  float* g = gebar + (size_t)p * EP;
  auto put = [&](int col, float v) { if (u) u[col] = v; g[col] = v; split16_put(u16, (size_t)p, col, v); };
  if (gl == 0) {
#pragma unroll
    for (int a = 0; a < 3; ++a) put(a, nb[a]);
    for (int col = E; col < EP; ++col) put(col, 0.f);
    for (int col = EP; col < ldu; ++col) { if (u) u[col] = 0.f; split16_put(u16, (size_t)p, col, 0.f); }
    return;
  }
  for (int k = gl - 1; k < multires; k += 7) {
    const float f = ldexpf(1.f, k);
#pragma unroll
    for (int a = 0; a < 3; ++a) {
      float sn, cs;
      sincosf(c[a] * scale * f, &sn, &cs);
      put(3 + 6 * k + a, f * cs * nb[a]);
      put(6 + 6 * k + a, -f * sn * nb[a]);
    }
  }
}

__global__ void k_fill_gebar(const float* __restrict__ gebar, int EP, int E, int64_t P, float* __restrict__ ubar,
                             int ldu, int col0, Split16 u16) {
  int64_t i = (int64_t)blockIdx.x * blockDim.x + threadIdx.x;
  if (i >= P * (int64_t)E) return;
  int64_t p = i / E;
  int e = (int)(i - p * E);
  float v = gebar[(size_t)p * EP + e] * kSqrtHalf;
  ubar[(size_t)p * ldu + col0 + e] = v;
  split16_put(u16, (size_t)p, col0 + e, v);
}

__global__ void k_heads_dgrad(const float* __restrict__ y6bar, const float* __restrict__ W6, int Hc,
                              const float* __restrict__ h, int64_t P, float* __restrict__ cbar, Split16 c16) {
  int64_t i4 = ((int64_t)blockIdx.x * blockDim.x + threadIdx.x) * 4;
  if (i4 >= P * (int64_t)Hc) return;
  int64_t p = i4 / Hc;
  int c = (int)(i4 - p * Hc);
  const float4 y0 = *reinterpret_cast<const float4*>(y6bar + (size_t)p * 8);
  const float4 y1 = *reinterpret_cast<const float4*>(y6bar + (size_t)p * 8 + 4);
  const float y[6] = {y0.x, y0.y, y0.z, y0.w, y1.x, y1.y};
  float acc[4] = {0.f, 0.f, 0.f, 0.f};
#pragma unroll
  for (int k = 0; k < 6; ++k) {
    const float4 w = *reinterpret_cast<const float4*>(W6 + (size_t)k * Hc + c);
    acc[0] = fmaf(y[k], w.x, acc[0]); acc[1] = fmaf(y[k], w.y, acc[1]);
    acc[2] = fmaf(y[k], w.z, acc[2]); acc[3] = fmaf(y[k], w.w, acc[3]);
  }
  const float4 hv = *reinterpret_cast<const float4*>(h + i4);
  float v[4] = {hv.x > 0.f ? acc[0] : 0.f, hv.y > 0.f ? acc[1] : 0.f, hv.z > 0.f ? acc[2] : 0.f, hv.w > 0.f ? acc[3] : 0.f};
  if (cbar) *reinterpret_cast<float4*>(cbar + i4) = make_float4(v[0], v[1], v[2], v[3]);
  split16_put4(c16, (size_t)p, c, v);
}

#define AVC_EPI_UNPACK float v[4] = {a.x, a.y, a.z, a.w}
#define AVC_EPI_DIRECT \
  __device__ __forceinline__ void operator()(int row, int col, float4 a) const { (*this)(row, col, a, prefetch(row, col)); }

__device__ __forceinline__ int clamp_group(int col, int n) { return max(0, min(col, (n - 4) & ~3)); }

__device__ __forceinline__ float4 load4_guarded(const float* p, int col, int N) {
  float4 r;
  r.x = col < N ? p[col] : 0.f; r.y = col + 1 < N ? p[col + 1] : 0.f;
  r.z = col + 2 < N ? p[col + 2] : 0.f; r.w = col + 3 < N ? p[col + 3] : 0.f;
  return r;
}

template <bool FAST>
struct EpiValue {
  static constexpr int kProbeId = 1;
  const float* bias; float* D1; int ldz; float* OUT; int ldo; float oscale; int N; Split16 o16;
  struct Aux { float4 b; };
  __device__ __forceinline__ Aux prefetch(int, int col) const { return {load4_guarded(bias, col, N)}; }
  __device__ __forceinline__ void operator()(int row, int col, float4 a, const Aux& x) const {
    AVC_EPI_UNPACK;
    const float bb[4] = {x.b.x, x.b.y, x.b.z, x.b.w};
    float dd[4], hh[4];
#pragma unroll
    for (int i = 0; i < 4; ++i) {
      softplus100_both<FAST>(v[i] + bb[i], &hh[i], &dd[i]);
      hh[i] *= oscale;
      if (col + i >= N) { hh[i] = 0.f; dd[i] = 0.f; }
    }
    if (D1) *reinterpret_cast<float4*>(D1 + (size_t)row * ldz + col) = make_float4(dd[0], dd[1], dd[2], dd[3]);
    if (col + 3 < N) {
      if (OUT) *reinterpret_cast<float4*>(OUT + (size_t)row * ldo + col) = make_float4(hh[0], hh[1], hh[2], hh[3]);
      split16_put4(o16, (size_t)row, col, hh);
    } else {
      for (int i = 0; i < 4 && col + i < N; ++i) {
        if (OUT) OUT[(size_t)row * ldo + col + i] = hh[i];
        split16_put(o16, (size_t)row, col + i, hh[i]);
      }
    }
  }
  AVC_EPI_DIRECT
};

struct EpiBias {
  static constexpr int kProbeId = 9;
  const float* bias; float* OUT; int ldo; int N; Split16 o16;
  struct Aux { float4 b; };
  __device__ __forceinline__ Aux prefetch(int, int col) const { return {load4_guarded(bias, col, N)}; }
  __device__ __forceinline__ void operator()(int row, int col, float4 a, const Aux& x) const {
    AVC_EPI_UNPACK;
    const float bb[4] = {x.b.x, x.b.y, x.b.z, x.b.w};
#pragma unroll
    for (int i = 0; i < 4; ++i) v[i] = (col + i < N) ? v[i] + bb[i] : 0.f;
    if (OUT) *reinterpret_cast<float4*>(OUT + (size_t)row * ldo + col) = make_float4(v[0], v[1], v[2], v[3]);
    split16_put4(o16, (size_t)row, col, v);
  }
  AVC_EPI_DIRECT
};

struct EpiChain {
  static constexpr int kProbeId = 2;
  int Nprev, Npp; float s; const float* D1prev; float* QTprev; float* GE; int EP; int E; Split16 q16;
  struct Aux { float4 d; };
  __device__ __forceinline__ Aux prefetch(int row, int col) const {
    const int c = clamp_group(col, Npp);
    return {*reinterpret_cast<const float4*>(D1prev + (size_t)row * Npp + c)};
  }
  using Stage = tc::Staged<4>;
  tc::StageOp stage_op(int) const { return {D1prev, Npp, Npp}; }
  static __device__ __forceinline__ Aux from_stage(const uint4 (&r)[1]) {
    return {make_float4(__uint_as_float(r[0].x), __uint_as_float(r[0].y), __uint_as_float(r[0].z), __uint_as_float(r[0].w))};
  }
  __device__ __forceinline__ void operator()(int row, int col, float4 a, const Aux& x) const {
    AVC_EPI_UNPACK;
    if (col + 3 < Nprev) {
      const size_t o = (size_t)row * Npp + col;
      float q[4] = {x.d.x * v[0] * s, x.d.y * v[1] * s, x.d.z * v[2] * s, x.d.w * v[3] * s};
      if (QTprev) *reinterpret_cast<float4*>(QTprev + o) = make_float4(q[0], q[1], q[2], q[3]);
      split16_put4(q16, (size_t)row, col, q);
      return;
    }
    const float dd[4] = {x.d.x, x.d.y, x.d.z, x.d.w};
#pragma unroll
    for (int i = 0; i < 4; ++i) {
      int c = col + i;
      if (c < Nprev) {
        float qv = dd[i] * v[i] * s;
        if (QTprev) QTprev[(size_t)row * Npp + c] = qv;
        split16_put(q16, (size_t)row, c, qv);
      } else {
        if (c < Npp) { if (QTprev) QTprev[(size_t)row * Npp + c] = 0.f; split16_put(q16, (size_t)row, c, 0.f); }
        int e = c - Nprev;
        if (e < E) atomicAdd(GE + (size_t)row * EP + e, v[i] * kSqrtHalf);
      }
    }
  }
  AVC_EPI_DIRECT
};

struct EpiGe {
  static constexpr int kProbeId = 10;
  float* GE; int EP; int E;
  struct Aux { float4 g; };
  __device__ __forceinline__ Aux prefetch(int row, int col) const {
    return {*reinterpret_cast<const float4*>(GE + (size_t)row * EP + clamp_group(col, EP))};
  }
  __device__ __forceinline__ void operator()(int row, int col, float4 a, const Aux& x) const {
    AVC_EPI_UNPACK;
    const float gg[4] = {x.g.x, x.g.y, x.g.z, x.g.w};
#pragma unroll
    for (int i = 0; i < 4; ++i)
      if (col + i < E) GE[(size_t)row * EP + col + i] = gg[i] + v[i];
  }
  AVC_EPI_DIRECT
};

struct EpiColor0 {
  static constexpr int kProbeId = 7;
  const float* bias; const float* cin; const float* WxT; int ldt; float* OUT; int ldo; Split16 o16;
  struct Aux { float4 c0, c1; };
  __device__ __forceinline__ Aux prefetch(int row, int) const {
    return {*reinterpret_cast<const float4*>(cin + (size_t)row * 8), *reinterpret_cast<const float4*>(cin + (size_t)row * 8 + 4)};
  }
  __device__ __forceinline__ void operator()(int row, int col, float4 a, const Aux& x) const {
    AVC_EPI_UNPACK;
    const float cj[6] = {x.c0.x, x.c0.y, x.c0.z, x.c0.w, x.c1.x, x.c1.y};
#pragma unroll
    for (int i = 0; i < 4; ++i) v[i] += bias[col + i];
#pragma unroll
    for (int j = 0; j < 6; ++j) {
      const float4 w = *reinterpret_cast<const float4*>(WxT + (size_t)j * ldt + col);
      v[0] = fmaf(cj[j], w.x, v[0]); v[1] = fmaf(cj[j], w.y, v[1]);
      v[2] = fmaf(cj[j], w.z, v[2]); v[3] = fmaf(cj[j], w.w, v[3]);
    }
#pragma unroll
    for (int i = 0; i < 4; ++i) v[i] = fmaxf(v[i], 0.f);
    if (OUT) *reinterpret_cast<float4*>(OUT + (size_t)row * ldo + col) = make_float4(v[0], v[1], v[2], v[3]);
    split16_put4(o16, (size_t)row, col, v);
  }
  AVC_EPI_DIRECT
};

struct EpiRelu {
  static constexpr int kProbeId = 5;
  const float* bias; float* OUT; int ldo; Split16 o16;
  struct Aux { float4 b; };
  __device__ __forceinline__ Aux prefetch(int, int col) const {
    return {make_float4(bias[col], bias[col + 1], bias[col + 2], bias[col + 3])};
  }
  __device__ __forceinline__ void operator()(int row, int col, float4 a, const Aux& x) const {
    AVC_EPI_UNPACK;
    v[0] = fmaxf(v[0] + x.b.x, 0.f); v[1] = fmaxf(v[1] + x.b.y, 0.f);
    v[2] = fmaxf(v[2] + x.b.z, 0.f); v[3] = fmaxf(v[3] + x.b.w, 0.f);
    if (OUT) *reinterpret_cast<float4*>(OUT + (size_t)row * ldo + col) = make_float4(v[0], v[1], v[2], v[3]);
    split16_put4(o16, (size_t)row, col, v);
  }
  AVC_EPI_DIRECT
};

struct EpiDgradRelu {
  static constexpr int kProbeId = 6;
  const float* Hm; const __nv_bfloat16* Hhi; float* OUT; int ld; Split16 o16;
  struct Aux { uint4 raw; };
  __device__ __forceinline__ Aux prefetch(int row, int col) const {
    if (Hm) return {*reinterpret_cast<const uint4*>(Hm + (size_t)row * ld + col)};
    const uint2 h = *reinterpret_cast<const uint2*>(Hhi + (size_t)row * o16.ld + col);
    return {make_uint4(h.x, h.y, 0u, 0u)};
  }
  __device__ __forceinline__ void l2_prefetch(int m0, int n0, int bn, int M, int et, int nth) const {
    if (Hm) tc::l2_prefetch_tile<4>(Hm, ld, ld, m0, n0, bn, M, et, nth);
    else tc::l2_prefetch_tile<2>(Hhi, o16.ld, o16.ld, m0, n0, bn, M, et, nth);
  }
  __device__ __forceinline__ void operator()(int row, int col, float4 a, const Aux& x) const {
    AVC_EPI_UNPACK;
    bool on[4];
    if (Hm) {
      on[0] = __uint_as_float(x.raw.x) > 0.f; on[1] = __uint_as_float(x.raw.y) > 0.f;
      on[2] = __uint_as_float(x.raw.z) > 0.f; on[3] = __uint_as_float(x.raw.w) > 0.f;
    } else {
      on[0] = (x.raw.x & 0x00007fffu) != 0u; on[1] = (x.raw.x & 0x7fff0000u) != 0u;
      on[2] = (x.raw.y & 0x00007fffu) != 0u; on[3] = (x.raw.y & 0x7fff0000u) != 0u;
    }
#pragma unroll
    for (int i = 0; i < 4; ++i) v[i] = on[i] ? v[i] : 0.f;
    if (OUT) *reinterpret_cast<float4*>(OUT + (size_t)row * ld + col) = make_float4(v[0], v[1], v[2], v[3]);
    split16_put4(o16, (size_t)row, col, v);
  }
  AVC_EPI_DIRECT
};

struct EpiStore {
  static constexpr int kProbeId = 8;
  float* OUT; int ldo; int N; Split16 o16;
  __device__ __forceinline__ void operator()(int row, int col, float4 a) const {
    AVC_EPI_UNPACK;
#pragma unroll
    for (int i = 0; i < 4; ++i) v[i] = (col + i < N) ? v[i] : 0.f;
    if (OUT) *reinterpret_cast<float4*>(OUT + (size_t)row * ldo + col) = make_float4(v[0], v[1], v[2], v[3]);
    split16_put4(o16, (size_t)row, col, v);
  }
};

struct EpiChainBwd {
  static constexpr int kProbeId = 3;
  int N, Np; const float* D1; const float* QT; Split16 qt16; float* ZBAR; float* UNEXT; int ldu; float s_next; Split16 u16;
  struct Aux { float4 d; uint4 q; };
  __device__ __forceinline__ Aux prefetch(int row, int col) const {
    const size_t o = (size_t)row * Np + clamp_group(col, Np);
    Aux x;
    x.d = *reinterpret_cast<const float4*>(D1 + o);
    if (QT) {
      x.q = *reinterpret_cast<const uint4*>(QT + o);
    } else {
      const size_t o16 = (size_t)row * qt16.ld + clamp_group(col, Np);
      const uint2 h = *reinterpret_cast<const uint2*>(qt16.hi + o16), l = *reinterpret_cast<const uint2*>(qt16.lo + o16);
      x.q = make_uint4(h.x, h.y, l.x, l.y);
    }
    return x;
  }
  using Stage = tc::Staged<4, 2, 2>;
  tc::StageOp stage_op(int i) const {
    if (QT || Np % 4 || N > Np) return {nullptr, 0, 0};
    return i == 0 ? tc::StageOp{D1, Np, Np} : tc::StageOp{i == 1 ? qt16.hi : qt16.lo, qt16.ld, Np};
  }
  static __device__ __forceinline__ Aux from_stage(const uint4 (&r)[3]) {
    return {make_float4(__uint_as_float(r[0].x), __uint_as_float(r[0].y), __uint_as_float(r[0].z), __uint_as_float(r[0].w)),
            make_uint4(r[1].x, r[1].y, r[2].x, r[2].y)};
  }
  __device__ __forceinline__ void operator()(int row, int col, float4 a, const Aux& x) const {
    AVC_EPI_UNPACK;
    const size_t o = (size_t)row * Np + col;
    const float dd[4] = {x.d.x, x.d.y, x.d.z, x.d.w};
    float qq[4];
    if (QT) { qq[0] = __uint_as_float(x.q.x); qq[1] = __uint_as_float(x.q.y); qq[2] = __uint_as_float(x.q.z); qq[3] = __uint_as_float(x.q.w); }
    else split16_get4(make_uint2(x.q.x, x.q.y), make_uint2(x.q.z, x.q.w), qq);
    float u[4], zb[4];
#pragma unroll
    for (int i = 0; i < 4; ++i) {
      u[i] = dd[i] * v[i] * s_next;
      zb[i] = kBeta * (1.f - dd[i]) * qq[i] * v[i];
    }
    if (UNEXT) *reinterpret_cast<float4*>(UNEXT + (size_t)row * ldu + col) = make_float4(u[0], u[1], u[2], u[3]);
    split16_put4(u16, (size_t)row, col, u);
    *reinterpret_cast<float4*>(ZBAR + o) = make_float4(zb[0], zb[1], zb[2], zb[3]);
  }
  AVC_EPI_DIRECT
};

struct EpiDgrad {
  static constexpr int kProbeId = 4;
  int Nprev, Npp; float s; const float* D1prev; float* ZBARprev; const float* sdfbar; const float* wsdf;
  float sdf_inv_scale; Split16 z16; int store_f32;
  struct Aux { float4 d, zb; };
  __device__ __forceinline__ Aux prefetch(int row, int col) const {
    const size_t o = (size_t)row * Npp + clamp_group(col, Npp);
    return {*reinterpret_cast<const float4*>(D1prev + o), *reinterpret_cast<const float4*>(ZBARprev + o)};
  }
  using Stage = tc::Staged<4, 4>;
  tc::StageOp stage_op(int i) const {
    if (Npp % 4 || Nprev > Npp) return {nullptr, 0, 0};
    return {i == 0 ? D1prev : ZBARprev, Npp, Npp};
  }
  static __device__ __forceinline__ Aux from_stage(const uint4 (&r)[2]) {
    return {make_float4(__uint_as_float(r[0].x), __uint_as_float(r[0].y), __uint_as_float(r[0].z), __uint_as_float(r[0].w)),
            make_float4(__uint_as_float(r[1].x), __uint_as_float(r[1].y), __uint_as_float(r[1].z), __uint_as_float(r[1].w))};
  }
  __device__ __forceinline__ void operator()(int row, int col, float4 a, const Aux& x) const {
    AVC_EPI_UNPACK;
    float sb = sdfbar ? sdfbar[row] * sdf_inv_scale : 0.f;
    const size_t o = (size_t)row * Npp + col;
    const float dd[4] = {x.d.x, x.d.y, x.d.z, x.d.w}, zo[4] = {x.zb.x, x.zb.y, x.zb.z, x.zb.w};
    float r[4];
#pragma unroll
    for (int i = 0; i < 4; ++i) {
      float ab = v[i];
      if (sdfbar) ab = fmaf(sb, wsdf[col + i], ab);
      r[i] = fmaf(dd[i], ab * s, zo[i]);
    }
    if (store_f32) *reinterpret_cast<float4*>(ZBARprev + o) = make_float4(r[0], r[1], r[2], r[3]);
    split16_put4(z16, (size_t)row, col, r);
  }
  AVC_EPI_DIRECT
};

struct CompositeArgs {
  const float* rays_d;
  const float* z_vals;
  const float* sdf;
  const float* cin;
  const float* rgb6;
  const float* background;
  int bg_kind;
  const float* ctx;
  float cos_anneal;
  float sample_dist;
  int S; int64_t Rc;
};

struct SampleTerms { float alpha, araw, Pp, Pn, ep, en, tc, dist, gn, relax; };

__device__ __forceinline__ SampleTerms sample_terms(const CompositeArgs& A, int64_t r, int j, float inv_s,
                                                    const float d[3]) {
  SampleTerms t;
  int64_t p = r * A.S + j;
  float z0 = A.z_vals[p];
  t.dist = (j + 1 < A.S) ? __fsub_rn(A.z_vals[p + 1], z0) : A.sample_dist;
  const float4 c0 = *reinterpret_cast<const float4*>(A.cin + (size_t)p * 8);
  const float4 c1 = *reinterpret_cast<const float4*>(A.cin + (size_t)p * 8 + 4);
  const float n0 = c0.w, n1 = c1.x, n2 = c1.y;
  float sdf = A.sdf[p];
  t.tc = d[0] * n0 + d[1] * n1 + d[2] * n2;
  float ic = -(fmaxf(-t.tc * 0.5f + 0.5f, 0.f) * (1.0f - A.cos_anneal) + fmaxf(-t.tc, 0.f) * A.cos_anneal);
  t.en = sdf + ic * t.dist * 0.5f;
  t.ep = sdf - ic * t.dist * 0.5f;
  t.Pp = sigmoidf_acc(t.ep * inv_s);
  t.Pn = sigmoidf_acc(t.en * inv_s);
  t.araw = (t.Pp - t.Pn + 1e-5f) / (t.Pp + 1e-5f);
  t.alpha = fminf(fmaxf(t.araw, 0.f), 1.f);
  t.gn = sqrtf(n0 * n0 + n1 * n1 + n2 * n2);
  float xn = sqrtf(c0.x * c0.x + c0.y * c0.y + c0.z * c0.z);
  t.relax = xn < 1.2f ? 1.f : 0.f;
  return t;
}

__device__ __forceinline__ float warp_excl_prod(float v, float* total) {
  const int lane = threadIdx.x & 31;
  float inc = v;
#pragma unroll
  for (int o = 1; o < 32; o <<= 1) {
    float t = __shfl_up_sync(0xffffffffu, inc, o);
    if (lane >= o) inc *= t;
  }
  *total = __shfl_sync(0xffffffffu, inc, 31);
  float ex = __shfl_up_sync(0xffffffffu, inc, 1);
  return lane == 0 ? 1.f : ex;
}

__global__ void __launch_bounds__(256)
k_composite_fwd(CompositeArgs A, float* __restrict__ color, float* __restrict__ extra, float* __restrict__ s_val,
                float* __restrict__ cdf, float* __restrict__ wsum_out, float* __restrict__ wmax_out,
                float* __restrict__ weights, float* __restrict__ ray_part) {
  const int64_t r = (int64_t)blockIdx.x * (blockDim.x >> 5) + (threadIdx.x >> 5);
  if (r >= A.Rc) return;
  const int lane = threadIdx.x & 31;
  const float inv_s = A.ctx[CTX_INV_S];
  const float d[3] = {A.rays_d[r * 3], A.rays_d[r * 3 + 1], A.rays_d[r * 3 + 2]};
  float carry = 1.f;
  float acc[6] = {0.f, 0.f, 0.f, 0.f, 0.f, 0.f};
  float wsum = 0.f, wmax = -1.f, eik_num = 0.f, eik_den = 0.f;
  for (int j0 = 0; j0 < A.S; j0 += 32) {
    const int j = j0 + lane;
    const bool ok = j < A.S;
    SampleTerms t;
    float one_m = 1.f;
    if (ok) {
      t = sample_terms(A, r, j, inv_s, d);
      one_m = 1.f - t.alpha + 1e-7f;
    }
    float total;
    float T = carry * warp_excl_prod(one_m, &total);
    carry *= total;
    if (ok) {
      const int64_t p = r * A.S + j;
      float w = t.alpha * T;
      weights[p] = w;
      cdf[p] = t.Pp;
      const float4 q0 = *reinterpret_cast<const float4*>(A.rgb6 + (size_t)p * 8);
      const float4 q1 = *reinterpret_cast<const float4*>(A.rgb6 + (size_t)p * 8 + 4);
      acc[0] += w * q0.x; acc[1] += w * q0.y; acc[2] += w * q0.z;
      acc[3] += w * q0.w; acc[4] += w * q1.x; acc[5] += w * q1.y;
      wsum += w;
      wmax = fmaxf(wmax, w);
      float e = t.gn - 1.f;
      eik_num += t.relax * e * e;
      eik_den += t.relax;
    }
  }
#pragma unroll
  for (int i = 0; i < 6; ++i) acc[i] = warp_sum(acc[i]);
  wsum = warp_sum(wsum); eik_num = warp_sum(eik_num); eik_den = warp_sum(eik_den);
#pragma unroll
  for (int o = 16; o > 0; o >>= 1) wmax = fmaxf(wmax, __shfl_xor_sync(0xffffffffu, wmax, o));
  if (lane == 0) {
    float bg[3] = {0.f, 0.f, 0.f};
    if (A.bg_kind == 1) { bg[0] = A.background[0]; bg[1] = A.background[1]; bg[2] = A.background[2]; }
    else if (A.bg_kind == 2) { bg[0] = bg[1] = bg[2] = A.background[r]; }
    color[r * 3 + 0] = acc[0]; color[r * 3 + 1] = acc[1]; color[r * 3 + 2] = acc[2];
    extra[r * 3 + 0] = acc[3] + bg[0] * (1.f - wsum);
    extra[r * 3 + 1] = acc[4] + bg[1] * (1.f - wsum);
    extra[r * 3 + 2] = acc[5] + bg[2] * (1.f - wsum);
    wsum_out[r] = wsum; wmax_out[r] = wmax;
    s_val[r] = 1.0f / inv_s;
    ray_part[r * 4 + 0] = eik_num; ray_part[r * 4 + 1] = eik_den;
  }
}

struct CompositeBwdArgs {
  const float* g_color; const float* g_extra; const float* g_wsum; const float* g_wmax;
  const float* g_w; const float* g_cdf; const float* g_n; const float* g_gerr;
  const float* weights;
  float* y6bar; float* sdfbar; float* nbar; float* ray_part;
};

__global__ void __launch_bounds__(256) k_composite_bwd(CompositeArgs A, CompositeBwdArgs G) {
  const int64_t r = (int64_t)blockIdx.x * (blockDim.x >> 5) + (threadIdx.x >> 5);
  if (r >= A.Rc) return;
  const int lane = threadIdx.x & 31;
  const float inv_s = A.ctx[CTX_INV_S];
  const float eik_den_total = A.ctx[CTX_EIK_DEN];
  const float g_gerr = G.g_gerr ? G.g_gerr[0] : 0.f;
  const float d[3] = {A.rays_d[r * 3], A.rays_d[r * 3 + 1], A.rays_d[r * 3 + 2]};
  float gc[6] = {0.f, 0.f, 0.f, 0.f, 0.f, 0.f};
  if (G.g_color) { gc[0] = G.g_color[r * 3]; gc[1] = G.g_color[r * 3 + 1]; gc[2] = G.g_color[r * 3 + 2]; }
  if (G.g_extra) { gc[3] = G.g_extra[r * 3]; gc[4] = G.g_extra[r * 3 + 1]; gc[5] = G.g_extra[r * 3 + 2]; }
  float wbar_common = G.g_wsum ? G.g_wsum[r] : 0.f;
  if (A.bg_kind == 1) wbar_common -= gc[3] * A.background[0] + gc[4] * A.background[1] + gc[5] * A.background[2];
  else if (A.bg_kind == 2) wbar_common -= (gc[3] + gc[4] + gc[5]) * A.background[r];
  const int nb = (A.S + 31) >> 5;

  int amax = -1;
  float g_wmax = 0.f;
  if (G.g_wmax) {
    g_wmax = G.g_wmax[r];
    float best = -1.f; int bi = 0x7fffffff;
    for (int j = lane; j < A.S; j += 32) {
      float w = G.weights[r * A.S + j];
      if (w > best) { best = w; bi = j; }
    }
#pragma unroll
    for (int o = 16; o > 0; o >>= 1) {
      float ob = __shfl_xor_sync(0xffffffffu, best, o);
      int oi = __shfl_xor_sync(0xffffffffu, bi, o);
      if (ob > best || (ob == best && oi < bi)) { best = ob; bi = oi; }
    }
    amax = bi;
  }

  SampleTerms tt[8];
  float Tj[8], wb[8], ww[8];
  float carry = 1.f;
#pragma unroll
  for (int b = 0; b < 8; ++b) {
    if (b >= nb) break;
    const int j = b * 32 + lane;
    const bool ok = j < A.S;
    float one_m = 1.f;
    if (ok) { tt[b] = sample_terms(A, r, j, inv_s, d); one_m = 1.f - tt[b].alpha + 1e-7f; }
    float total;
    float T = carry * warp_excl_prod(one_m, &total);
    carry *= total;
    Tj[b] = T; wb[b] = 0.f; ww[b] = 0.f;
    if (ok) {
      const int64_t p = r * A.S + j;
      float w = tt[b].alpha * T;
      ww[b] = w;
      const float4 q0 = *reinterpret_cast<const float4*>(A.rgb6 + (size_t)p * 8);
      const float4 q1 = *reinterpret_cast<const float4*>(A.rgb6 + (size_t)p * 8 + 4);
      float wbar = wbar_common + (G.g_w ? G.g_w[p] : 0.f);
      wbar += gc[0] * q0.x + gc[1] * q0.y + gc[2] * q0.z + gc[3] * q0.w + gc[4] * q1.x + gc[5] * q1.y;
      if (j == amax) wbar += g_wmax;
      wb[b] = wbar;
      float y[6] = {q0.x, q0.y, q0.z, q0.w, q1.x, q1.y};
      float o6[8];
#pragma unroll
      for (int i = 0; i < 6; ++i) o6[i] = w * gc[i] * y[i] * (1.f - y[i]);
      o6[6] = o6[7] = 0.f;
      reinterpret_cast<float4*>(G.y6bar + (size_t)p * 8)[0] = make_float4(o6[0], o6[1], o6[2], o6[3]);
      reinterpret_cast<float4*>(G.y6bar + (size_t)p * 8)[1] = make_float4(o6[4], o6[5], 0.f, 0.f);
    }
  }
  float invs_bar = 0.f;
  float suffix_carry = 0.f;
#pragma unroll
  for (int b = 7; b >= 0; --b) {
    if (b >= nb) continue;
    const int j = b * 32 + lane;
    const bool ok = j < A.S;
    float v = ok ? wb[b] * ww[b] : 0.f;
    float inc = v;
#pragma unroll
    for (int o = 1; o < 32; o <<= 1) {
      float t = __shfl_down_sync(0xffffffffu, inc, o);
      if (lane + o < 32) inc += t;
    }
    float block_total = __shfl_sync(0xffffffffu, inc, 0);
    float Asuf = inc - v + suffix_carry;
    suffix_carry += block_total;
    if (ok) {
      const SampleTerms& t = tt[b];
      const int64_t p = r * A.S + j;
      float abar = wb[b] * Tj[b] - Asuf / (1.f - t.alpha + 1e-7f);
      if (!(t.araw >= 0.f && t.araw <= 1.f)) abar = 0.f;
      float den = t.Pp + 1e-5f;
      float Ppbar = abar * t.Pn / (den * den) + (G.g_cdf ? G.g_cdf[p] : 0.f);
      float Pnbar = -abar / den;
      float dPp = t.Pp * (1.f - t.Pp), dPn = t.Pn * (1.f - t.Pn);
      float epbar = Ppbar * dPp * inv_s, enbar = Pnbar * dPn * inv_s;
      invs_bar += Ppbar * dPp * t.ep + Pnbar * dPn * t.en;
      G.sdfbar[p] = epbar + enbar;
      float icbar = (enbar - epbar) * t.dist * 0.5f;
// ... 119 lines not shown
```

### avatarclip_b200/csrc/avc_tc.cu

```cuda
#include "avc_gemm_tc.cuh"

using namespace avc;

namespace {
struct EpiPlainStore {
  float* C; int ldc; int N;
  __device__ void operator()(int row, int col, float4 a) const {
    float v[4] = {a.x, a.y, a.z, a.w};
    for (int i = 0; i < 4 && col + i < N; ++i) C[(size_t)row * ldc + col + i] = v[i];
  }
};
}

extern "C" {

int avc_tc_gemm_nt_test(const float* A, const float* B, int64_t M, int32_t N, int32_t K, int32_t nprod, float* C,
                        void* workspace, size_t workspace_bytes, avc_stream_t stream) {
  if (!A || !B || !C || !workspace) return AVC_E_NULL;
  if (M <= 0 || N <= 0 || K <= 0 || (nprod != 1 && nprod != 3)) return AVC_E_SIZE;
  const int ld = (int)round_up(K, 8);
  Carver cv(workspace);
  __nv_bfloat16* ah = cv.take<__nv_bfloat16>(M * ld);
  __nv_bfloat16* al = cv.take<__nv_bfloat16>(M * ld);
  __nv_bfloat16* bh = cv.take<__nv_bfloat16>((int64_t)N * ld);
  __nv_bfloat16* bl = cv.take<__nv_bfloat16>((int64_t)N * ld);
  if (cv.used() > workspace_bytes) return AVC_E_SIZE;
  cudaStream_t st = (cudaStream_t)stream;
  tc::k_split_bf16<<<(int)((M * ld + 255) / 256), 256, 0, st>>>(A, M, K, K, ah, al, ld);
  tc::k_split_bf16<<<(int)(((int64_t)N * ld + 255) / 256), 256, 0, st>>>(B, N, K, K, bh, bl, ld);
  AVC_LAUNCH_TRY();
  tc::SplitPtr a{ah, al, ld}, b{bh, bl, ld};
  EpiPlainStore e{C, N, N};
  if (nprod == 3) return tc::launch_gemm_tc_nt<3, EpiPlainStore>(st, M, N, K, a, b, e);
  return tc::launch_gemm_tc_nt<1, EpiPlainStore>(st, M, N, K, a, b, e);
}

int avc_tc_gemm_tn_test(const float* A, const float* B, int64_t P, int32_t N1, int32_t N2, int32_t nprod, float* C,
                        float* colsum, void* workspace, size_t workspace_bytes, avc_stream_t stream) {
  if (!A || !B || !C || !workspace) return AVC_E_NULL;
  if (P <= 0 || N1 <= 0 || N2 <= 0 || (nprod != 1 && nprod != 3)) return AVC_E_SIZE;
  const int l1 = (int)round_up(N1, 8), l2 = (int)round_up(N2, 8);
  Carver cv(workspace);
  __nv_bfloat16* ah = cv.take<__nv_bfloat16>(P * l1);
  __nv_bfloat16* al = cv.take<__nv_bfloat16>(P * l1);
  __nv_bfloat16* bh = cv.take<__nv_bfloat16>(P * l2);
  __nv_bfloat16* bl = cv.take<__nv_bfloat16>(P * l2);
  if (cv.used() > workspace_bytes) return AVC_E_SIZE;
  cudaStream_t st = (cudaStream_t)stream;
  tc::k_split_bf16<<<(int)((P * l1 + 255) / 256), 256, 0, st>>>(A, P, N1, N1, ah, al, l1);
  tc::k_split_bf16<<<(int)((P * l2 + 255) / 256), 256, 0, st>>>(B, P, N2, N2, bh, bl, l2);
  AVC_LAUNCH_TRY();
  tc::SplitPtr a{ah, al, l1}, b{bh, bl, l2};
  if (nprod == 3) return tc::launch_gemm_tc_tn<3>(st, P, N1, N2, a, b, C, N2, colsum);
  return tc::launch_gemm_tc_tn<1>(st, P, N1, N2, a, b, C, N2, colsum);
}

}
```

### include/avc_b200.h

```cpp
#ifndef AVC_B200_H
#define AVC_B200_H

#include <stddef.h>
#include <stdint.h>

#ifdef __cplusplus
extern "C" {
#endif

typedef void* avc_stream_t;

#define AVC_OK 0
#define AVC_E_BADCFG (-1)
#define AVC_E_NULL (-2)
#define AVC_E_SIZE (-3)
#define AVC_E_ALIGN (-4)
#define AVC_E_NOSTASH (-5)

#define AVC_ABI_VERSION 3
int avc_abi_version(void);
const char* avc_build_arch(void);

typedef struct avc_neus_cfg {
  int32_t sdf_d_in;
  int32_t sdf_d_out;
  int32_t sdf_d_hidden;
  int32_t sdf_n_layers;
  uint32_t sdf_skip_mask;
  int32_t sdf_multires;
  float sdf_scale;
  int32_t col_d_feature;
  int32_t col_d_hidden;
  int32_t col_n_layers;
  int32_t n_samples;
  int32_t n_importance;
  int32_t up_sample_steps;
  int32_t engine;
  int32_t color_products;
  int32_t wgrad_products;
} avc_neus_cfg;

int avc_neus_param_count(const avc_neus_cfg* cfg, int64_t* n_params);
int avc_neus_param_offset(const avc_neus_cfg* cfg, int net, int layer, int which, int64_t* offset,
                          int64_t* numel);

int avc_neus_workspace_bytes(const avc_neus_cfg* cfg, int64_t max_rays_per_chunk, size_t* bytes);

typedef struct avc_neus_outputs {
  float* color_fine;
  float* extra_color_fine;
  float* s_val;
  float* cdf_fine;
  float* weight_sum;
  float* weight_max;
  float* gradients;
  float* weights;
  float* mid_z_vals;
  float* gradient_error;
  float* inside_sphere;
  float* z_vals;
} avc_neus_outputs;

int avc_neus_render_fwd(const avc_neus_cfg* cfg, const float* params, const float* rays_o,
                        const float* rays_d, const float* near, const float* far,
                        const float* jitter, const float* background, int bg_kind,
                        const float* z_vals_in, float cos_anneal_ratio, int64_t R,
                        const avc_neus_outputs* out, void* workspace, size_t workspace_bytes,
                        int64_t max_rays_per_chunk, avc_stream_t stream);

typedef struct avc_neus_cotangents {
  const float* color_fine;
  const float* extra_color_fine;
  const float* s_val;
  const float* cdf_fine;
  const float* weight_sum;
  const float* weight_max;
  const float* gradients;
  const float* weights;
  const float* gradient_error;
} avc_neus_cotangents;

int avc_neus_render_bwd(const avc_neus_cfg* cfg, const float* params, const float* rays_o,
                        const float* rays_d, const float* background, int bg_kind,
                        float cos_anneal_ratio, int64_t R, const avc_neus_outputs* fwd_out,
                        const avc_neus_cotangents* cot, float* grad_params, void* workspace,
                        size_t workspace_bytes, int64_t max_rays_per_chunk, int32_t flags,
                        avc_stream_t stream);
#define AVC_BWD_RECOMPUTE 1

int avc_neus_sdf_query(const avc_neus_cfg* cfg, const float* params, const float* pts, int64_t P,
                       float* sdf_out, void* workspace, size_t workspace_bytes,
                       avc_stream_t stream);


typedef struct avc_clip_cfg {
  int32_t image_size;
  int32_t patch;
  int32_t width;
  int32_t layers;
  int32_t heads;
  int32_t mlp;
  int32_t out_dim;
} avc_clip_cfg;

typedef struct avc_clip_layer_weights {
  const float *ln1_g, *ln1_b, *ln2_g, *ln2_b;
  const void *w_qkv, *w_qkv_t;
  const float* b_qkv;
  const void *w_out, *w_out_t;
  const float* b_out;
  const void *w_fc, *w_fc_t;
  const float* b_fc;
  const void *w_proj, *w_proj_t;
  const float* b_proj;
} avc_clip_layer_weights;

#define AVC_CLIP_MAX_LAYERS 24
typedef struct avc_clip_weights {
  const void *w_patch, *w_patch_t;
  const float *cls, *pos;
  const float *ln_pre_g, *ln_pre_b, *ln_post_g, *ln_post_b;
  const float* proj;
  avc_clip_layer_weights layer[AVC_CLIP_MAX_LAYERS];
} avc_clip_weights;

int avc_clip_workspace_bytes(const avc_clip_cfg* cfg, int32_t B, size_t* bytes);

int avc_clip_loss_fwd(const avc_clip_cfg* cfg, const avc_clip_weights* w, const float* canvases,
                      int32_t H, int32_t W, int32_t B, int32_t input_mode, const float* text_emb,
                      float* emb_out, float* cos_out, void* workspace, size_t workspace_bytes,
                      avc_stream_t stream);
int avc_clip_loss_bwd(const avc_clip_cfg* cfg, const avc_clip_weights* w, int32_t H, int32_t W, int32_t B,
                      int32_t input_mode, const float* text_emb, const float* g_cos, const float* g_emb,
                      float* d_canvases, void* workspace, size_t workspace_bytes, avc_stream_t stream);

typedef struct avc_clip_text_cfg {
  int32_t context;
  int32_t vocab;
  int32_t width;
  int32_t layers;
  int32_t heads;
  int32_t mlp;
  int32_t out_dim;
} avc_clip_text_cfg;

typedef struct avc_clip_text_weights {
  const float* token_emb;
  const float* pos;
  const float *ln_final_g, *ln_final_b;
  const float* proj;
  avc_clip_layer_weights layer[AVC_CLIP_MAX_LAYERS];
} avc_clip_text_weights;

int avc_clip_text_workspace_bytes(const avc_clip_text_cfg* cfg, int32_t B, size_t* bytes);
int avc_clip_encode_text(const avc_clip_text_cfg* cfg, const avc_clip_text_weights* w, const int32_t* tokens, int32_t B,
                         float* emb_out, void* workspace, size_t workspace_bytes, avc_stream_t stream);

typedef struct avc_loss_inputs {
  const float* color_fine;
  const float* extra_color_fine;
  const float* gradients;
  const float* weights;
  const float* weight_sum;
  const float* gradient_error;
  const int32_t* pix;
  const uint8_t* in_mask;
  const float* true_rgb;
  const float* mask;
  const float* background;
  int32_t bg_choice;
  float light_dir[3];
  float ambience;
  const float* view_scalars;
  float igr_weight, mask_weight, clip_weight;
  int32_t R, S, H, W;
  int32_t plain_texture;
  int32_t no_shading_term;
} avc_loss_inputs;

#define AVC_LOSS_SCALARS 16
int avc_loss_stage_fwd(const avc_loss_inputs* in, float* canvases, float* scalars, avc_stream_t stream);
int avc_loss_stage_bwd(const avc_loss_inputs* in, const float* d_canvases, const float* scalars,
                       const avc_neus_cotangents* cot_out, avc_stream_t stream);

int avc_neus_sdf_eval(const avc_neus_cfg* cfg, const float* params, const float* pts, int64_t P, float* sdf_feat_out,
                      float* grad_out, void* workspace, size_t workspace_bytes, avc_stream_t stream);

int avc_adam_step(float* params, const float* grads, float* exp_avg, float* exp_avg_sq, int64_t n,
                  float lr, float beta1, float beta2, float eps, int64_t step, float grad_scale,
                  avc_stream_t stream);
int avc_adam_step_dev(float* params, const float* grads, float* exp_avg, float* exp_avg_sq, int64_t n,
                      float* state, float beta1, float beta2, float eps, float grad_scale, avc_stream_t stream);

int avc_gen_rays(const float* pose_c2w, float fx, float fy, float cx, float cy, int32_t full_w, int32_t full_h,
                 int32_t W, int32_t H, const int32_t* pix, int32_t R, float* rays_o, float* rays_d, float* near,
                 float* far, avc_stream_t stream);

int avc_lbs_workspace_bytes(int32_t n_joints, size_t* bytes);
int avc_lbs_fwd(const float* v_shaped, const float* pose, int32_t pose2rot, const float* J_regressor,
                const int32_t* parents, const float* posedirs, const float* lbs_weights, int32_t V,
                int32_t n_joints, float* verts_out, float* joints_out, void* workspace,
                size_t workspace_bytes, avc_stream_t stream);

int avc_nearest_vertex(const float* query, int32_t N, const float* ref, int32_t M, int32_t* nearest,
                       avc_stream_t stream);

int avc_mesh_components_workspace_bytes(int32_t V, size_t* bytes);
int avc_mesh_components(const int32_t* faces, int32_t F, int32_t V, int32_t* labels, int32_t* kept, void* workspace,
                        size_t workspace_bytes, avc_stream_t stream);

int avc_lbs_rel_transforms(const float* v_template, const float* J_regressor, const int32_t* parents, int32_t V,
                           int32_t n_joints, const float* pose, int32_t pose2rot, int32_t n_frames, float* joints_out,
                           float* A_out, avc_stream_t stream);

int avc_inv_lbs(const float* verts, const int32_t* nearest, int32_t N, const float* lbs_weights, int32_t M,
                int32_t n_joints, const float* A, float* tpose_out, avc_stream_t stream);

int avc_lbs_frames(const float* tpose, const int32_t* nearest, int32_t N, const float* lbs_weights, int32_t M,
                   int32_t n_joints, const float* A, int32_t n_frames, int32_t frame_begin, int32_t frame_count,
                   float* out, avc_stream_t stream);

int avc_nearest_vertex_f32(const float* query, int32_t N, const float* ref, int32_t M, int32_t* nearest,
                           avc_stream_t stream);

int avc_mesh_cluster_workspace_bytes(int32_t V, int32_t F, size_t* bytes);
int avc_mesh_cluster(const float* verts, const uint8_t* colors, int32_t V, const int32_t* tris, int32_t F,
                     int32_t resolution, float* verts_out, float* colors_out, int32_t* tris_out, int32_t* counts,
                     void* workspace, size_t workspace_bytes, avc_stream_t stream);

int avc_tc_gemm_nt_test(const float* A, const float* B, int64_t M, int32_t N, int32_t K, int32_t nprod,
                        float* C, void* workspace, size_t workspace_bytes, avc_stream_t stream);
int avc_tc_gemm_tn_test(const float* A, const float* B, int64_t P, int32_t N1, int32_t N2, int32_t nprod,
                        float* C, float* colsum, void* workspace, size_t workspace_bytes, avc_stream_t stream);
int avc_tc_epi_test(int32_t kind, const float* A, const float* B, int64_t M, int32_t N, int32_t K, int32_t Nv,
                    const float* X, float* Y, int32_t ldx, const float* v1, const float* v2, float s, float s2, float* OUT,
                    float* OUT2, int32_t ld2, void* workspace, size_t workspace_bytes, avc_stream_t stream);
int avc_neus_kernel_test(int32_t kind, const int64_t* dims, const float* fscal, const void* const* in, void* const* out,
                         avc_stream_t stream);
int avc_clip_kernel_test(int32_t kind, const int32_t* dims, const void* const* in, void* const* out,
                         avc_stream_t stream);

int avc_raster_workspace_bytes(int32_t V, int32_t image_size, int32_t supersample, size_t* bytes);
int avc_raster_template(const float* verts, const int32_t* faces, int32_t V, int32_t F, const float* eye,
                        const float* at, int32_t image_size, int32_t supersample, float* rgb_out, uint8_t* mask_out,
                        void* workspace, size_t workspace_bytes, avc_stream_t stream);
int avc_dilate_count(const uint8_t* mask, int32_t n, int32_t iterations, uint8_t* dilated, int32_t* count_out,
                     avc_stream_t stream);
int avc_mask_compact(const uint8_t* dilated, int32_t n, int32_t W, int32_t cap, uint8_t* in_mask, int32_t* pix,
                     int32_t* count_out, avc_stream_t stream);
int avc_view_targets(const float* rgb, int32_t n, int32_t W, int32_t threshold_mask, float* true_rgb, float* mask,
                     avc_stream_t stream);
int avc_background_field(int32_t kind, int32_t H, int32_t W, uint32_t seed, int32_t chess_len, float sigma,
                         float* canvas_bg, const int32_t* pix, int32_t R, float* ray_bg, avc_stream_t stream);
int avc_uniform_fill(uint32_t seed, int32_t n, float lo, float hi, float* out, avc_stream_t stream);

int avc_chain_debug_read(long long* out8);
int avc_nt_probe_read(unsigned long long* host_out, int reset);

int avc_march_count(const float* field, int32_t nx, int32_t ny, int32_t nz, float iso, int32_t* counts,
                    avc_stream_t stream);
int avc_march_emit(const float* field, int32_t nx, int32_t ny, int32_t nz, float iso, const int32_t* offsets,
                   float* verts, int64_t* keys, avc_stream_t stream);

#ifdef __cplusplus
}
#endif
#endif
```

Baseline: 96.78.

## Stage GEMM epilogue outputs in swizzled shared memory and store them with TMA

Adds a ring-store epilogue path for the NT tensor-core GEMM. Epilogue functors that declare an Out layout write f32 and split-bf16 results into swizzled shared-memory slots, and the warp then issues bulk TMA tensor stores, replacing scattered per-thread global stores. It also removes the explicit L2 prefetch of epilogue operand tiles and enlarges the tensor-map cache. In exchange it reduces the epilogue batch width, uses shared memory for output slots that may cut pipeline stages, and adds bulk-group waits on slot reuse.

```diff
diff --git a/avatarclip_b200/csrc/avc_gemm_tc.cuh b/avatarclip_b200/csrc/avc_gemm_tc.cuh
--- a/avatarclip_b200/csrc/avc_gemm_tc.cuh
+++ b/avatarclip_b200/csrc/avc_gemm_tc.cuh
@@ -33,7 +33,7 @@
     if (spins > (1u << 26)) __trap();
   }
 }
-constexpr int kNtProbeSlots = 9;
+constexpr int kNtProbeSlots = 10;
 #ifdef AVC_NT_PROBE
 static __device__ unsigned long long g_nt_probe[16][kNtProbeSlots];
 #define AVC_PROBE(...) __VA_ARGS__
@@ -81,6 +81,14 @@
 __device__ __forceinline__ void tma_prefetch_desc(const CUtensorMap* map) {
   asm volatile("prefetch.tensormap [%0];" ::"l"((uint64_t)map) : "memory");
 }
+__device__ __forceinline__ void tma_store_2d(const CUtensorMap* map, uint32_t src, int x, int y) {
+  asm volatile("cp.async.bulk.tensor.2d.global.shared::cta.bulk_group [%0, {%2, %3}], [%1];"
+               ::"l"((uint64_t)map), "r"(src), "r"(x), "r"(y) : "memory");
+}
+__device__ __forceinline__ void bulk_commit() { asm volatile("cp.async.bulk.commit_group;" ::: "memory"); }
+template <int N>
+__device__ __forceinline__ void bulk_wait_read() { asm volatile("cp.async.bulk.wait_group.read %0;" ::"n"(N) : "memory"); }
+__device__ __forceinline__ void bulk_wait_all() { asm volatile("cp.async.bulk.wait_group 0;" ::: "memory"); }
 
 typedef CUresult (*PFN_encodeTiled)(CUtensorMap*, CUtensorMapDataType, cuuint32_t, void*, const cuuint64_t*,
                                     const cuuint64_t*, const cuuint32_t*, const cuuint32_t*, CUtensorMapInterleave,
@@ -129,9 +137,9 @@
 
 static inline int make_map_rows_cached(CUtensorMap* m, int es, const void* base, uint64_t rows, uint64_t cols,
                                        uint64_t ld, uint32_t box_cols, uint32_t box_rows) {
-  static thread_local MapCacheEntry cache[64];
+  static thread_local MapCacheEntry cache[256];
   const uint64_t h = ((uintptr_t)base >> 8) * 0x9E3779B97F4A7C15ull ^ (rows * 31 + cols * 131 + ld * 7 + box_cols + 3 * box_rows + es);
-  MapCacheEntry& e = cache[(h >> 32) & 63];
+  MapCacheEntry& e = cache[(h >> 32) & 255];
   const uint32_t bc = box_cols | ((uint32_t)es << 16);
   if (e.base == base && e.rows == rows && e.cols == cols && e.ld == ld && e.bc == bc && e.br == box_rows) {
     *m = e.map;
@@ -200,16 +208,20 @@
   using Aux = NoAux;
   static __device__ __forceinline__ Aux prefetch(const E&, int, int) { return {}; }
   static __device__ __forceinline__ void apply(const E& e, int r, int c, float4 a, const Aux&) { e(r, c, a); }
+  template <typename S>
+  static __device__ __forceinline__ void ring(const E& e, int r, int c, float4 a, const Aux&, const S& s) { e.ring(r, c, a, s); }
 };
 template <typename E>
 struct EpiTraits<E, std::void_t<typename E::Aux>> {
   using Aux = typename E::Aux;
   static __device__ __forceinline__ Aux prefetch(const E& e, int r, int c) { return e.prefetch(r, c); }
   static __device__ __forceinline__ void apply(const E& e, int r, int c, float4 a, const Aux& x) { e(r, c, a, x); }
-};
-template <typename E>
+  template <typename S>
+  static __device__ __forceinline__ void ring(const E& e, int r, int c, float4 a, const Aux& x, const S& s) { e.ring(r, c, a, x, s); }
+};
+template <typename E, bool RING = false>
 struct EpiBatch {
-  static constexpr int kB = sizeof(typename EpiTraits<E>::Aux) > 16 ? 2 : 4;
+  static constexpr int kB = (RING || sizeof(typename EpiTraits<E>::Aux) > 16) ? 2 : 4;
   static constexpr int kCols = 8 * kB;
 };
 
@@ -235,11 +247,15 @@
 template <>
 struct EpiMaps<0> {};
 template <int ES, int COLS>
-__device__ __forceinline__ uint4 stage_read(uint32_t slab, int r, int c) {
+__device__ __forceinline__ uint32_t box_addr(uint32_t slab, int r, int c) {
   constexpr int kSpan = COLS * ES;
   static_assert(kSpan == 32 || kSpan == 64 || kSpan == 128, "swizzle span");
   const uint32_t lin = (uint32_t)(r * kSpan + c * ES);
-  const uint32_t addr = slab + (lin ^ (((lin >> 7) & (kSpan / 16 - 1)) << 4));
+  return slab + (lin ^ (((lin >> 7) & (kSpan / 16 - 1)) << 4));
+}
+template <int ES, int COLS>
+__device__ __forceinline__ uint4 stage_read(uint32_t slab, int r, int c) {
+  const uint32_t addr = box_addr<ES, COLS>(slab, r, c);
   uint4 v = make_uint4(0u, 0u, 0u, 0u);
   if constexpr (ES == 4)
     asm volatile("ld.shared.v4.u32 {%0, %1, %2, %3}, [%4];" : "=r"(v.x), "=r"(v.y), "=r"(v.z), "=r"(v.w) : "r"(addr));
@@ -247,25 +263,56 @@
     asm volatile("ld.shared.v2.u32 {%0, %1}, [%2];" : "=r"(v.x), "=r"(v.y) : "r"(addr));
   return v;
 }
-template <int ES>
-__device__ __forceinline__ void l2_prefetch_tile(const void* base, int ld, int ncols, int m0, int n0, int bn, int M,
-                                                 int et, int nth) {
-  constexpr int kPerLine = 128 / ES;
-  const int lpr = (bn + kPerLine - 1) / kPerLine;
-  for (int i = et; i < kNtBM * lpr; i += nth) {
-    const int row = m0 + i / lpr, col = n0 + (i % lpr) * kPerLine;
-    if (row < M && col < ncols)
-      asm volatile("prefetch.global.L2 [%0];" ::"l"(reinterpret_cast<const char*>(base) + ((size_t)row * ld + col) * ES));
-  }
-}
+
+template <int... ES>
+struct Outs {
+  static constexpr int kN = sizeof...(ES);
+  static constexpr int kColBytes = (ES + ...);
+  __host__ __device__ static constexpr int es(int i) { int k = 0, r = 0; ((r = (k++ == i ? ES : r)), ...); return r; }
+  __host__ __device__ static constexpr int before(int i) { int k = 0, r = 0; ((r += (k++ < i ? ES : 0)), ...); return r; }
+};
+struct OutOp { const void* base; int ld; int cols; };
 template <typename E, typename = void>
-struct EpiL2 {
-  static __device__ __forceinline__ void run(const E&, int, int, int, int, int, int) {}
+struct EpiOut {
+  static constexpr int kN = 0, kSlotBytes = 0;
 };
 template <typename E>
-struct EpiL2<E, std::void_t<decltype(&E::l2_prefetch)>> {
-  static __device__ __forceinline__ void run(const E& e, int m0, int n0, int bn, int M, int et, int nth) {
-    if (m0 < M) e.l2_prefetch(m0, n0, bn, M, et, nth);
+struct EpiOut<E, std::void_t<typename E::Out>> {
+  using O = typename E::Out;
+  static_assert(EpiStage<E>::kN == 0, "a functor stages its operands or ring-stores its outputs, not both");
+  static constexpr int kN = O::kN, kSlotBytes = kNtBM * EpiBatch<E, true>::kCols * O::kColBytes;
+};
+template <int N>
+struct EpiOutMaps { CUtensorMap m[N]; };
+template <>
+struct EpiOutMaps<0> {};
+template <typename O, int COLS>
+struct RingSink {
+  uint32_t box; int r, c; uint32_t mask;
+  __device__ __forceinline__ uint32_t at(int i) const {
+    const uint32_t slab = box + 16 * COLS * O::before(i);
+    return O::es(i) == 4 ? box_addr<4, COLS>(slab, r, c) : box_addr<2, COLS>(slab, r, c);
+  }
+  __device__ __forceinline__ void f32(int i, const float v[4]) const {
+    if (!((mask >> i) & 1u)) return;
+    asm volatile("st.shared.v4.f32 [%0], {%1, %2, %3, %4};" ::"r"(at(i)), "f"(v[0]), "f"(v[1]), "f"(v[2]), "f"(v[3]) : "memory");
+  }
+  __device__ __forceinline__ void split(int i, const float v[4]) const {
+    if (!((mask >> i) & 3u)) return;
+    const uint32_t h01 = bf16x2_bits(v[0], v[1]), h23 = bf16x2_bits(v[2], v[3]);
+    const float r0 = v[0] - __uint_as_float(h01 << 16), r1 = v[1] - __uint_as_float(h01 & 0xffff0000u);
+    const float r2 = v[2] - __uint_as_float(h23 << 16), r3 = v[3] - __uint_as_float(h23 & 0xffff0000u);
+    if ((mask >> i) & 1u) asm volatile("st.shared.v2.u32 [%0], {%1, %2};" ::"r"(at(i)), "r"(h01), "r"(h23) : "memory");
+    if ((mask >> (i + 1)) & 1u)
+      asm volatile("st.shared.v2.u32 [%0], {%1, %2};" ::"r"(at(i + 1)), "r"(bf16x2_bits(r0, r1)), "r"(bf16x2_bits(r2, r3)) : "memory");
+  }
+  __device__ __forceinline__ void zero() const {
+#pragma unroll
+    for (int i = 0; i < O::kN; ++i) {
+      if (!((mask >> i) & 1u)) continue;
+      if (O::es(i) == 4) asm volatile("st.shared.v4.u32 [%0], {%1, %1, %1, %1};" ::"r"(at(i)), "r"(0u) : "memory");
+      else asm volatile("st.shared.v2.u32 [%0], {%1, %1};" ::"r"(at(i)), "r"(0u) : "memory");
+    }
   }
 };
 
@@ -274,13 +321,16 @@
   uint32_t full0, empty0;
   int q0;
   int r, c;
-};
-template <int BN, int SLOTS, typename Epi, typename MmaDone>
+  int m0, n0, wq;
+  uint32_t omask;
+};
+template <int BN, int SLOTS, bool RING, typename Epi, typename OMaps, typename MmaDone>
 __device__ __forceinline__ void epilogue_nt(const Epi& epi, const float (&acc)[BN / 2], int row, int col0, int M, int N,
-                                            int lane, MmaDone&& mma_done, const EpiRing& ring, long long& w_stage) {
+                                            int lane, MmaDone&& mma_done, const EpiRing& ring, const OMaps& omaps,
+                                            long long& w_stage, long long& w_drain) {
   using Tr = EpiTraits<Epi>;
   const bool odd = lane & 1;
-  constexpr int kB = EpiBatch<Epi>::kB, kNB = BN / 8 / kB;
+  constexpr int kB = EpiBatch<Epi, RING>::kB, kNB = BN / 8 / kB;
   auto group = [&](int j) {
     const float s0 = odd ? acc[4 * j] : acc[4 * j + 2], s1 = odd ? acc[4 * j + 1] : acc[4 * j + 3];
     const float r0 = __shfl_xor_sync(0xffffffffu, s0, 1), r1 = __shfl_xor_sync(0xffffffffu, s1, 1);
@@ -317,6 +367,50 @@
       __syncwarp();
       if ((lane & 31) == 0) mbar_arrive(ring.empty0 + 8 * s);
     }
+  } else if constexpr (RING) {
+    using O = typename Epi::Out;
+    constexpr int kCols = EpiBatch<Epi, true>::kCols, kSlot = EpiOut<Epi>::kSlotBytes, kWarpBytes = 16 * kCols * O::kColBytes;
+    typename Tr::Aux aux[2][kB];
+    auto load = [&](int b) {
+#pragma unroll
+      for (int u = 0; u < kB; ++u) {
+        const int col = col0 + 8 * (kB * b + u);
+        if (row < M && col < N) aux[b & 1][u] = Tr::prefetch(epi, row, col);
+      }
+    };
+    load(0);
+    mma_done();
+#pragma unroll
+    for (int b = 0; b < kNB; ++b) {
+      if (b + 1 < kNB) load(b + 1);
+      const uint32_t box = ring.base + ((ring.q0 + b) % SLOTS) * kSlot + ring.wq * kWarpBytes;
+      if (lane == 0) {
+        AVC_PROBE(const long long t0 = clock64());
+        bulk_wait_read<SLOTS - 1>();
+        AVC_PROBE(w_drain += clock64() - t0);
+      }
+      __syncwarp();
+#pragma unroll
+      for (int u = 0; u < kB; ++u) {
+        const int j = kB * b + u;
+        const float4 v = group(j);
+        const int col = col0 + 8 * j;
+        const RingSink<O, kCols> sink{box, ring.r - 16 * ring.wq, ring.c + 8 * u, ring.omask};
+        if (row < M) {
+          if (col < N) Tr::ring(epi, row, col, v, aux[b & 1][u], sink);
+          else sink.zero();
+        }
+      }
+      fence_proxy_async();
+      __syncwarp();
+      if (lane == 0) {
+#pragma unroll
+        for (int i = 0; i < O::kN; ++i)
+          if ((ring.omask >> i) & 1u)
+            tma_store_2d(&omaps.m[i], box + 16 * kCols * O::before(i), ring.n0 + b * kCols, ring.m0 + 16 * ring.wq);
+        bulk_commit();
+      }
+    }
   } else {
     typename Tr::Aux aux[2][kB];
     auto load = [&](int b) {
@@ -344,14 +438,16 @@
   }
 }
 
-template <int BN, int NPROD, bool RESB, typename Epi>
+template <int BN, int NPROD, bool RESB, typename Epi, bool RING = false>
 __global__ void __launch_bounds__(kNtThreads, 1)
 gemm_tc_nt_kernel(const __grid_constant__ CUtensorMap mapAhi, const __grid_constant__ CUtensorMap mapAlo,
                   const __grid_constant__ CUtensorMap mapBhi, const __grid_constant__ CUtensorMap mapBlo,
-                  int M, int N, int K, Epi epi, int b_const, const __grid_constant__ EpiMaps<EpiStage<Epi>::kN> emaps) {
-  using Cfg = TcCfg<BN, NPROD, RESB, EpiStage<Epi>::kSlotBytes>;
+                  int M, int N, int K, Epi epi, int b_const, const __grid_constant__ EpiMaps<EpiStage<Epi>::kN> emaps,
+                  const __grid_constant__ EpiOutMaps<EpiOut<Epi>::kN> omaps, uint32_t omask) {
+  static_assert(!RING || EpiOut<Epi>::kN > 0, "only functors with an Out ring-store");
+  using Cfg = TcCfg<BN, NPROD, RESB, RING ? EpiOut<Epi>::kSlotBytes : EpiStage<Epi>::kSlotBytes>;
   constexpr int kStaged = EpiStage<Epi>::kN;
-  constexpr int kEpiCols = EpiBatch<Epi>::kCols, kEpiNB = BN / kEpiCols;
+  constexpr int kEpiCols = EpiBatch<Epi, RING>::kCols, kEpiNB = BN / kEpiCols;
   extern __shared__ uint8_t smem_raw[];
   uint8_t* smem = (uint8_t*)(((uintptr_t)smem_raw + 1023) & ~(uintptr_t)1023);
   constexpr int kOpBytes = Cfg::STAGES * Cfg::STAGE_BYTES + Cfg::BRES_BYTES + Cfg::EPI_BYTES;
@@ -378,6 +474,10 @@
     if constexpr (kStaged > 0) {
       for (int i = 0; i < kStaged; ++i) tma_prefetch_desc(&emaps.m[i]);
       for (int s = 0; s < 2 * Cfg::EPI_SLOTS; ++s) { mbar_init(efull0 + 8 * s, 1); mbar_init(eempty0 + 8 * s, 4); }
+    }
+    if constexpr (RING) {
+      for (int i = 0; i < EpiOut<Epi>::kN; ++i)
+        if ((omask >> i) & 1u) tma_prefetch_desc(&omaps.m[i]);
     }
     fence_barrier_init();
   }
@@ -449,14 +549,12 @@
   const int row_in = 16 * wq + (lane >> 2) + 8 * (lane & 1), col_in = 4 * ((lane >> 1) & 1);
   pdl_wait();
   float acc[BN / 2];
-  long long w_stage = 0;
+  long long w_stage = 0, w_drain = 0;
   EpiRing ring{smem_base + kEpiOff + c * Cfg::EPI_SLOTS * Cfg::SLOT_BYTES, efull0 + 8 * c * Cfg::EPI_SLOTS,
-               eempty0 + 8 * c * Cfg::EPI_SLOTS, 0, row_in, col_in};
+               eempty0 + 8 * c * Cfg::EPI_SLOTS, 0, row_in, col_in, 0, n0, wq, omask};
   AVC_PROBE(long long w_full = 0, w_turn = 0, t_mma = 0, t_epi = 0; const long long t_loop0 = clock64());
-  EpiL2<Epi>::run(epi, (m_first + c * m_stride) * kNtBM, n0, BN, M, tw, 128);
   for (int j = c; j < n_tiles; j += 2) {
     const int m0 = (m_first + j * m_stride) * kNtBM;
-    EpiL2<Epi>::run(epi, m0 + 2 * m_stride * kNtBM, n0, BN, M, tw, 128);
     AVC_PROBE(const long long t_turn0 = clock64());
     if (j > 0) named_bar_sync(kNtTurnBar + c, 256);
     AVC_PROBE(const long long t_mma0 = clock64(); w_turn += t_mma0 - t_turn0);
@@ -490,7 +588,8 @@
     }
     if (j + 1 < n_tiles) named_bar_arrive(kNtTurnBar + (c ^ 1), 256);
     ring.q0 = (j >> 1) * kEpiNB;
-    epilogue_nt<BN, Cfg::EPI_SLOTS>(epi, acc, m0 + row_in, n0 + col_in, M, N, lane, [&] {
+    ring.m0 = m0;
+    epilogue_nt<BN, Cfg::EPI_SLOTS, RING>(epi, acc, m0 + row_in, n0 + col_in, M, N, lane, [&] {
       wgmma_wait<0>();
       wgmma_fence_acc(acc);
       if (leader) {
@@ -498,12 +597,16 @@
         mbar_arrive(empty0 + 8 * last);
       }
       AVC_PROBE(t_mma += clock64() - t_mma0);
-    }, ring, w_stage);
+    }, ring, omaps, w_stage, w_drain);
     AVC_PROBE(t_epi += clock64() - t_mma0);
   }
-  (void)w_stage;
+  if constexpr (RING) {
+    if (lane == 0) bulk_wait_all();
+  }
+  (void)w_stage; (void)w_drain;
   AVC_PROBE(if (leader) {
     AVC_PROBE_ADD(EpiProbeId<Epi>::value, 8, w_stage);
+    AVC_PROBE_ADD(EpiProbeId<Epi>::value, 9, w_drain);
     AVC_PROBE_ADD(EpiProbeId<Epi>::value, 2, w_full);
     AVC_PROBE_ADD(EpiProbeId<Epi>::value, 3, w_turn);
     AVC_PROBE_ADD(EpiProbeId<Epi>::value, 4, t_mma);
@@ -512,10 +615,40 @@
   })
 }
 
+template <int BN, int NPROD, bool RESB, typename Epi, bool RING>
+static inline int launch_gemm_tc_nt_kern(cudaStream_t st, int64_t M, int N, int K, const CUtensorMap (&mab)[4],
+                                         const Epi& epi, bool b_const, const EpiMaps<EpiStage<Epi>::kN>& emaps,
+                                         const EpiOutMaps<EpiOut<Epi>::kN>& omaps, uint32_t omask) {
+  using Cfg = TcCfg<BN, NPROD, RESB, RING ? EpiOut<Epi>::kSlotBytes : EpiStage<Epi>::kSlotBytes>;
+  auto kern = gemm_tc_nt_kernel<BN, NPROD, RESB, Epi, RING>;
+  static thread_local bool attr_set = false;
+  if (!attr_set) {
+    AVC_CUDA_TRY(cudaFuncSetAttribute(kern, cudaFuncAttributeMaxDynamicSharedMemorySize, Cfg::SMEM_BYTES));
+    attr_set = true;
+  }
+  static thread_local int num_sms = 0;
+  if (!num_sms) {
+    int dev = 0;
+    AVC_CUDA_TRY(cudaGetDevice(&dev));
+    AVC_CUDA_TRY(cudaDeviceGetAttribute(&num_sms, cudaDevAttrMultiProcessorCount, dev));
+  }
+  const int tiles_n = ceil_div(N, BN);
+  const int ntiles = ceil_div(M, kNtBM) * tiles_n;
+  int g = ntiles < num_sms ? ntiles : num_sms;
+  g = (g / tiles_n) * tiles_n;
+  if (g < tiles_n) return AVC_E_BADCFG;
+  dim3 grid(g);
+  AVC_CUDA_TRY(launch_pdl(kern, dim3(grid), dim3(kNtThreads), (size_t)Cfg::SMEM_BYTES, st, mab[0], mab[1], mab[2], mab[3],
+                          (int)M, N, K, epi, b_const ? 1 : 0, emaps, omaps, omask));
+  AVC_LAUNCH_TRY();
+  return 0;
+}
+
+inline thread_local int g_nt_last_ring = -1;
+
 template <int BN, int NPROD, bool RESB, typename Epi>
 static inline int launch_gemm_tc_nt_bn(cudaStream_t st, int64_t M, int N, int K, const SplitPtr& A, const SplitPtr& B,
                                        const Epi& epi, bool b_const) {
-  using Cfg = TcCfg<BN, NPROD, RESB, EpiStage<Epi>::kSlotBytes>;
   EpiMaps<EpiStage<Epi>::kN> emaps;
   if constexpr (EpiStage<Epi>::kN > 0) {
     for (int i = 0; i < EpiStage<Epi>::kN; ++i) {
@@ -525,36 +658,35 @@
                                    (uint64_t)op.ld, EpiBatch<Epi>::kCols, kNtBM));
     }
   }
-  CUtensorMap mAh, mAl, mBh, mBl;
-  AVC_TRY(make_map_bf16_cached(&mAh, A.hi, (uint64_t)M, (uint64_t)K, (uint64_t)A.ld, kBK, kNtBM));
-  AVC_TRY(make_map_bf16_cached(&mBh, B.hi, (uint64_t)N, (uint64_t)K, (uint64_t)B.ld, kBK, BN));
+  EpiOutMaps<EpiOut<Epi>::kN> omaps{};
+  uint32_t omask = 0;
+  bool ring = false;
+  if constexpr (EpiOut<Epi>::kN > 0) {
+    ring = true;
+    for (int i = 0; i < EpiOut<Epi>::kN; ++i) {
+      const OutOp op = epi.out_op(i, N);
+      if (!op.base) continue;
+      const int es = Epi::Out::es(i);
+      if (((uintptr_t)op.base & 15u) || (op.ld * es) % 16 || (op.cols * es) % 16) { ring = false; break; }
+      AVC_TRY(make_map_rows_cached(&omaps.m[i], Epi::Out::es(i), op.base, (uint64_t)M, (uint64_t)op.cols,
+                                   (uint64_t)op.ld, EpiBatch<Epi, true>::kCols, 16));
+      omask |= 1u << i;
+    }
+  }
+  CUtensorMap mab[4];
+  AVC_TRY(make_map_bf16_cached(&mab[0], A.hi, (uint64_t)M, (uint64_t)K, (uint64_t)A.ld, kBK, kNtBM));
+  AVC_TRY(make_map_bf16_cached(&mab[2], B.hi, (uint64_t)N, (uint64_t)K, (uint64_t)B.ld, kBK, BN));
   if (NPROD == 3) {
-    AVC_TRY(make_map_bf16_cached(&mAl, A.lo, (uint64_t)M, (uint64_t)K, (uint64_t)A.ld, kBK, kNtBM));
-    AVC_TRY(make_map_bf16_cached(&mBl, B.lo, (uint64_t)N, (uint64_t)K, (uint64_t)B.ld, kBK, BN));
+    AVC_TRY(make_map_bf16_cached(&mab[1], A.lo, (uint64_t)M, (uint64_t)K, (uint64_t)A.ld, kBK, kNtBM));
+    AVC_TRY(make_map_bf16_cached(&mab[3], B.lo, (uint64_t)N, (uint64_t)K, (uint64_t)B.ld, kBK, BN));
   } else {
-    mAl = mAh; mBl = mBh;
-  }
-  auto kern = gemm_tc_nt_kernel<BN, NPROD, RESB, Epi>;
-  static thread_local bool attr_set = false;
-  if (!attr_set) {
-    AVC_CUDA_TRY(cudaFuncSetAttribute(kern, cudaFuncAttributeMaxDynamicSharedMemorySize, Cfg::SMEM_BYTES));
-    attr_set = true;
-  }
-  static thread_local int num_sms = 0;
-  if (!num_sms) {
-    int dev = 0;
-    AVC_CUDA_TRY(cudaGetDevice(&dev));
-    AVC_CUDA_TRY(cudaDeviceGetAttribute(&num_sms, cudaDevAttrMultiProcessorCount, dev));
-  }
-  const int tiles_n = ceil_div(N, BN);
-  const int ntiles = ceil_div(M, kNtBM) * tiles_n;
-  int g = ntiles < num_sms ? ntiles : num_sms;
-  g = (g / tiles_n) * tiles_n;
-  if (g < tiles_n) return AVC_E_BADCFG;
-  dim3 grid(g);
-  AVC_CUDA_TRY(launch_pdl(kern, dim3(grid), dim3(kNtThreads), (size_t)Cfg::SMEM_BYTES, st, mAh, mAl, mBh, mBl, (int)M, N, K, epi, b_const ? 1 : 0, emaps));
-  AVC_LAUNCH_TRY();
-  return 0;
+    mab[1] = mab[0]; mab[3] = mab[2];
+  }
+  g_nt_last_ring = ring ? 1 : 0;
+  if constexpr (EpiOut<Epi>::kN > 0) {
+    if (ring) return launch_gemm_tc_nt_kern<BN, NPROD, RESB, Epi, true>(st, M, N, K, mab, epi, b_const, emaps, omaps, omask);
+  }
+  return launch_gemm_tc_nt_kern<BN, NPROD, RESB, Epi, false>(st, M, N, K, mab, epi, b_const, emaps, omaps, 0);
 }
 
 template <int NPROD, typename Epi>
diff --git a/avatarclip_b200/csrc/avc_neus.cu b/avatarclip_b200/csrc/avc_neus.cu
--- a/avatarclip_b200/csrc/avc_neus.cu
+++ b/avatarclip_b200/csrc/avc_neus.cu
@@ -596,14 +596,15 @@
   __nv_bfloat16* al = cv.take<__nv_bfloat16>(M * ld);
   __nv_bfloat16* bh = cv.take<__nv_bfloat16>((int64_t)N * ld);
   __nv_bfloat16* bl = cv.take<__nv_bfloat16>((int64_t)N * ld);
-  __nv_bfloat16* xh = cv.take<__nv_bfloat16>(M * ldx);
-  __nv_bfloat16* xl = cv.take<__nv_bfloat16>(M * ldx);
+  const int ldm = kind % 100 == 11 ? 2 * ld2 : ldx;
+  __nv_bfloat16* xh = cv.take<__nv_bfloat16>(M * ldm);
+  __nv_bfloat16* xl = cv.take<__nv_bfloat16>(M * ldm);
   if (cv.used() > workspace_bytes) return AVC_E_SIZE;
   cudaStream_t st = (cudaStream_t)stream;
   tc::k_split_bf16<<<blocks_for(M * ld, 256), 256, 0, st>>>(A, M, K, K, ah, al, ld);
   tc::k_split_bf16<<<blocks_for((int64_t)N * ld, 256), 256, 0, st>>>(B, N, K, K, bh, bl, ld);
   const float* xs = kind == 0 ? Y : X;
-  if (kind == 0 || kind == 4) tc::k_split_bf16<<<blocks_for(M * ldx, 256), 256, 0, st>>>(xs, M, ldx, ldx, xh, xl, ldx);
+  if (kind == 0 || kind == 4 || kind % 100 == 11) tc::k_split_bf16<<<blocks_for(M * ldm, 256), 256, 0, st>>>(xs, M, ldx, ldx, xh, xl, ldm);
   AVC_LAUNCH_TRY();
   const tc::SplitPtr a{ah, al, ld}, b{bh, bl, ld};
   const Split16 none{nullptr, nullptr, ldx};
@@ -635,6 +636,41 @@
     case 5: {
       EpiGe e{OUT2, ld2, N};
       return tc::launch_gemm_tc_nt<3>(st, M, N, K, a, b, e);
+    }
+  }
+  const bool np1 = kind >= 108 && kind <= 111;
+  if (np1) kind -= 100;
+  if (kind < 6 || kind > 11) return AVC_E_BADCFG;
+  auto launch_color = [&](const auto& e) {
+    return np1 ? tc::launch_gemm_tc_nt<1>(st, M, N, K, a, b, e) : tc::launch_gemm_tc_nt<3>(st, M, N, K, a, b, e);
+  };
+  if (!OUT2 || (!v1 && kind != 10 && kind != 11)) return AVC_E_NULL;
+  __nv_bfloat16* o16 = reinterpret_cast<__nv_bfloat16*>(OUT2);
+  const Split16 split{o16, o16 + ld2, 2 * ld2};
+  switch (kind) {
+    case 6: {
+      EpiValue<true> e{v1, Y, ldx, OUT, ldx, s, N, split};
+      return tc::launch_gemm_tc_nt<3>(st, M, N, K, a, b, e);
+    }
+    case 7: {
+      EpiBias e{v1, OUT, ldx, N, split};
+      return tc::launch_gemm_tc_nt<3>(st, M, N, K, a, b, e);
+    }
+    case 8: {
+      EpiColor0 e{v1, X, v2, ldx, OUT, ldx, split};
+      return launch_color(e);
+    }
+    case 9: {
+      EpiRelu e{v1, OUT, ldx, split};
+      return launch_color(e);
+    }
+    case 10: {
+      EpiStore e{OUT, ldx, N, split};
+      return launch_color(e);
+    }
+    case 11: {
+      EpiDgradRelu e{nullptr, xh, OUT, ldx, Split16{o16, o16 + ld2, 2 * ld2}};
+      return launch_color(e);
     }
   }
   return AVC_E_BADCFG;
diff --git a/avatarclip_b200/csrc/avc_neus_kernels.cuh b/avatarclip_b200/csrc/avc_neus_kernels.cuh
--- a/avatarclip_b200/csrc/avc_neus_kernels.cuh
+++ b/avatarclip_b200/csrc/avc_neus_kernels.cuh
@@ -604,6 +604,11 @@
 #define AVC_EPI_DIRECT \
   __device__ __forceinline__ void operator()(int row, int col, float4 a) const { (*this)(row, col, a, prefetch(row, col)); }
 
+inline tc::OutOp epi_group_out(int i, float* out, int ldo, const Split16& s, int n) {
+  const int cols = (n + 3) & ~3;
+  return i == 0 ? tc::OutOp{out, ldo, cols} : tc::OutOp{i == 1 ? s.hi : s.lo, s.ld, cols};
+}
+
 __device__ __forceinline__ int clamp_group(int col, int n) { return max(0, min(col, (n - 4) & ~3)); }
 
 __device__ __forceinline__ float4 load4_guarded(const float* p, int col, int N) {
@@ -619,16 +624,30 @@
   const float* bias; float* D1; int ldz; float* OUT; int ldo; float oscale; int N; Split16 o16;
   struct Aux { float4 b; };
   __device__ __forceinline__ Aux prefetch(int, int col) const { return {load4_guarded(bias, col, N)}; }
-  __device__ __forceinline__ void operator()(int row, int col, float4 a, const Aux& x) const {
+  __device__ __forceinline__ void vals(int col, float4 a, const Aux& x, float hh[4], float dd[4]) const {
     AVC_EPI_UNPACK;
     const float bb[4] = {x.b.x, x.b.y, x.b.z, x.b.w};
-    float dd[4], hh[4];
 #pragma unroll
     for (int i = 0; i < 4; ++i) {
       softplus100_both<FAST>(v[i] + bb[i], &hh[i], &dd[i]);
       hh[i] *= oscale;
       if (col + i >= N) { hh[i] = 0.f; dd[i] = 0.f; }
     }
+  }
+  using Out = tc::Outs<4, 4, 2, 2>;
+  tc::OutOp out_op(int i, int) const {
+    return i == 0 ? tc::OutOp{D1, ldz, ldz} : i == 1 ? tc::OutOp{OUT, ldo, N}
+                                                     : tc::OutOp{i == 2 ? o16.hi : o16.lo, o16.ld, N};
+  }
+  template <typename S>
+  __device__ __forceinline__ void ring(int, int col, float4 a, const Aux& x, const S& s) const {
+    float dd[4], hh[4];
+    vals(col, a, x, hh, dd);
+    s.f32(0, dd); s.f32(1, hh); s.split(2, hh);
+  }
+  __device__ __forceinline__ void operator()(int row, int col, float4 a, const Aux& x) const {
+    float dd[4], hh[4];
+    vals(col, a, x, hh, dd);
     if (D1) *reinterpret_cast<float4*>(D1 + (size_t)row * ldz + col) = make_float4(dd[0], dd[1], dd[2], dd[3]);
     if (col + 3 < N) {
       if (OUT) *reinterpret_cast<float4*>(OUT + (size_t)row * ldo + col) = make_float4(hh[0], hh[1], hh[2], hh[3]);
@@ -648,11 +667,22 @@
   const float* bias; float* OUT; int ldo; int N; Split16 o16;
   struct Aux { float4 b; };
   __device__ __forceinline__ Aux prefetch(int, int col) const { return {load4_guarded(bias, col, N)}; }
+  __device__ __forceinline__ void vals(int col, float4 a, const Aux& x, float v[4]) const {
+    const float aa[4] = {a.x, a.y, a.z, a.w}, bb[4] = {x.b.x, x.b.y, x.b.z, x.b.w};
+#pragma unroll
+    for (int i = 0; i < 4; ++i) v[i] = (col + i < N) ? aa[i] + bb[i] : 0.f;
+  }
+  using Out = tc::Outs<4, 2, 2>;
+  tc::OutOp out_op(int i, int n) const { return epi_group_out(i, OUT, ldo, o16, n); }
+  template <typename S>
+  __device__ __forceinline__ void ring(int, int col, float4 a, const Aux& x, const S& s) const {
+    float v[4];
+    vals(col, a, x, v);
+    s.f32(0, v); s.split(1, v);
+  }
   __device__ __forceinline__ void operator()(int row, int col, float4 a, const Aux& x) const {
-    AVC_EPI_UNPACK;
-    const float bb[4] = {x.b.x, x.b.y, x.b.z, x.b.w};
-#pragma unroll
-    for (int i = 0; i < 4; ++i) v[i] = (col + i < N) ? v[i] + bb[i] : 0.f;
+    float v[4];
+    vals(col, a, x, v);
     if (OUT) *reinterpret_cast<float4*>(OUT + (size_t)row * ldo + col) = make_float4(v[0], v[1], v[2], v[3]);
     split16_put4(o16, (size_t)row, col, v);
   }
@@ -713,6 +743,13 @@
     for (int i = 0; i < 4; ++i)
       if (col + i < E) GE[(size_t)row * EP + col + i] = gg[i] + v[i];
   }
+  using Out = tc::Outs<4>;
+  tc::OutOp out_op(int, int) const { return {GE, EP, EP}; }
+  template <typename S>
+  __device__ __forceinline__ void ring(int, int, float4 a, const Aux& x, const S& s) const {
+    const float v[4] = {x.g.x + a.x, x.g.y + a.y, x.g.z + a.z, x.g.w + a.w};
+    s.f32(0, v);
+  }
   AVC_EPI_DIRECT
 };
 
@@ -723,8 +760,8 @@
   __device__ __forceinline__ Aux prefetch(int row, int) const {
     return {*reinterpret_cast<const float4*>(cin + (size_t)row * 8), *reinterpret_cast<const float4*>(cin + (size_t)row * 8 + 4)};
   }
-  __device__ __forceinline__ void operator()(int row, int col, float4 a, const Aux& x) const {
-    AVC_EPI_UNPACK;
+  __device__ __forceinline__ void vals(int col, float4 a, const Aux& x, float v[4]) const {
+    v[0] = a.x; v[1] = a.y; v[2] = a.z; v[3] = a.w;
     const float cj[6] = {x.c0.x, x.c0.y, x.c0.z, x.c0.w, x.c1.x, x.c1.y};
 #pragma unroll
     for (int i = 0; i < 4; ++i) v[i] += bias[col + i];
@@ -736,6 +773,10 @@
     }
 #pragma unroll
     for (int i = 0; i < 4; ++i) v[i] = fmaxf(v[i], 0.f);
+  }
+  __device__ __forceinline__ void operator()(int row, int col, float4 a, const Aux& x) const {
+    float v[4];
+    vals(col, a, x, v);
     if (OUT) *reinterpret_cast<float4*>(OUT + (size_t)row * ldo + col) = make_float4(v[0], v[1], v[2], v[3]);
     split16_put4(o16, (size_t)row, col, v);
   }
@@ -749,10 +790,21 @@
   __device__ __forceinline__ Aux prefetch(int, int col) const {
     return {make_float4(bias[col], bias[col + 1], bias[col + 2], bias[col + 3])};
   }
+  __device__ __forceinline__ static void vals(float4 a, const Aux& x, float v[4]) {
+    v[0] = fmaxf(a.x + x.b.x, 0.f); v[1] = fmaxf(a.y + x.b.y, 0.f);
+    v[2] = fmaxf(a.z + x.b.z, 0.f); v[3] = fmaxf(a.w + x.b.w, 0.f);
+  }
+  using Out = tc::Outs<4, 2, 2>;
+  tc::OutOp out_op(int i, int n) const { return epi_group_out(i, OUT, ldo, o16, n); }
+  template <typename S>
+  __device__ __forceinline__ void ring(int, int, float4 a, const Aux& x, const S& s) const {
+    float v[4];
+    vals(a, x, v);
+    s.f32(0, v); s.split(1, v);
+  }
   __device__ __forceinline__ void operator()(int row, int col, float4 a, const Aux& x) const {
-    AVC_EPI_UNPACK;
-    v[0] = fmaxf(v[0] + x.b.x, 0.f); v[1] = fmaxf(v[1] + x.b.y, 0.f);
-    v[2] = fmaxf(v[2] + x.b.z, 0.f); v[3] = fmaxf(v[3] + x.b.w, 0.f);
+    float v[4];
+    vals(a, x, v);
     if (OUT) *reinterpret_cast<float4*>(OUT + (size_t)row * ldo + col) = make_float4(v[0], v[1], v[2], v[3]);
     split16_put4(o16, (size_t)row, col, v);
   }
@@ -768,12 +820,22 @@
     const uint2 h = *reinterpret_cast<const uint2*>(Hhi + (size_t)row * o16.ld + col);
     return {make_uint4(h.x, h.y, 0u, 0u)};
   }
-  __device__ __forceinline__ void l2_prefetch(int m0, int n0, int bn, int M, int et, int nth) const {
-    if (Hm) tc::l2_prefetch_tile<4>(Hm, ld, ld, m0, n0, bn, M, et, nth);
-    else tc::l2_prefetch_tile<2>(Hhi, o16.ld, o16.ld, m0, n0, bn, M, et, nth);
+  using Out = tc::Outs<4, 2, 2>;
+  tc::OutOp out_op(int i, int n) const { return epi_group_out(i, OUT, ld, o16, n); }
+  template <typename S>
+  __device__ __forceinline__ void ring(int, int, float4 a, const Aux& x, const S& s) const {
+    float v[4];
+    vals(a, x, v);
+    s.f32(0, v); s.split(1, v);
   }
   __device__ __forceinline__ void operator()(int row, int col, float4 a, const Aux& x) const {
-    AVC_EPI_UNPACK;
+    float v[4];
+    vals(a, x, v);
+    if (OUT) *reinterpret_cast<float4*>(OUT + (size_t)row * ld + col) = make_float4(v[0], v[1], v[2], v[3]);
+    split16_put4(o16, (size_t)row, col, v);
+  }
+  __device__ __forceinline__ void vals(float4 a, const Aux& x, float v[4]) const {
+    v[0] = a.x; v[1] = a.y; v[2] = a.z; v[3] = a.w;
     bool on[4];
     if (Hm) {
       on[0] = __uint_as_float(x.raw.x) > 0.f; on[1] = __uint_as_float(x.raw.y) > 0.f;
@@ -784,8 +846,6 @@
     }
 #pragma unroll
     for (int i = 0; i < 4; ++i) v[i] = on[i] ? v[i] : 0.f;
-    if (OUT) *reinterpret_cast<float4*>(OUT + (size_t)row * ld + col) = make_float4(v[0], v[1], v[2], v[3]);
-    split16_put4(o16, (size_t)row, col, v);
   }
   AVC_EPI_DIRECT
 };
@@ -793,10 +853,22 @@
 struct EpiStore {
   static constexpr int kProbeId = 8;
   float* OUT; int ldo; int N; Split16 o16;
+  __device__ __forceinline__ void vals(int col, float4 a, float v[4]) const {
+    const float aa[4] = {a.x, a.y, a.z, a.w};
+#pragma unroll
+    for (int i = 0; i < 4; ++i) v[i] = (col + i < N) ? aa[i] : 0.f;
+  }
+  using Out = tc::Outs<4, 2, 2>;
+  tc::OutOp out_op(int i, int n) const { return epi_group_out(i, OUT, ldo, o16, n); }
+  template <typename S>
+  __device__ __forceinline__ void ring(int, int col, float4 a, const S& s) const {
+    float v[4];
+    vals(col, a, v);
+    s.f32(0, v); s.split(1, v);
+  }
   __device__ __forceinline__ void operator()(int row, int col, float4 a) const {
-    AVC_EPI_UNPACK;
-#pragma unroll
-    for (int i = 0; i < 4; ++i) v[i] = (col + i < N) ? v[i] : 0.f;
+    float v[4];
+    vals(col, a, v);
     if (OUT) *reinterpret_cast<float4*>(OUT + (size_t)row * ldo + col) = make_float4(v[0], v[1], v[2], v[3]);
     split16_put4(o16, (size_t)row, col, v);
   }
diff --git a/avatarclip_b200/csrc/avc_tc.cu b/avatarclip_b200/csrc/avc_tc.cu
--- a/avatarclip_b200/csrc/avc_tc.cu
+++ b/avatarclip_b200/csrc/avc_tc.cu
@@ -8,6 +8,13 @@
   __device__ void operator()(int row, int col, float4 a) const {
     float v[4] = {a.x, a.y, a.z, a.w};
     for (int i = 0; i < 4 && col + i < N; ++i) C[(size_t)row * ldc + col + i] = v[i];
+  }
+  using Out = tc::Outs<4>;
+  tc::OutOp out_op(int, int) const { return {C, ldc, N}; }
+  template <typename S>
+  __device__ void ring(int, int, float4 a, const S& s) const {
+    const float v[4] = {a.x, a.y, a.z, a.w};
+    s.f32(0, v);
   }
 };
 }
@@ -55,4 +62,6 @@
   return tc::launch_gemm_tc_tn<1>(st, P, N1, N2, a, b, C, N2, colsum);
 }
 
+int avc_tc_nt_last_ring(void) { return tc::g_nt_last_ring; }
+
 }
diff --git a/include/avc_b200.h b/include/avc_b200.h
--- a/include/avc_b200.h
+++ b/include/avc_b200.h
@@ -232,6 +232,7 @@
                         float* C, void* workspace, size_t workspace_bytes, avc_stream_t stream);
 int avc_tc_gemm_tn_test(const float* A, const float* B, int64_t P, int32_t N1, int32_t N2, int32_t nprod,
                         float* C, float* colsum, void* workspace, size_t workspace_bytes, avc_stream_t stream);
+int avc_tc_nt_last_ring(void);
 int avc_tc_epi_test(int32_t kind, const float* A, const float* B, int64_t M, int32_t N, int32_t K, int32_t Nv,
                     const float* X, float* Y, int32_t ldx, const float* v1, const float* v2, float s, float s2, float* OUT,
                     float* OUT2, int32_t ld2, void* workspace, size_t workspace_bytes, avc_stream_t stream);
```

Measured after the change: 100.8, median of 6. +4.1%, better.
